# YooSungHyun/RNNTransducer

Measured on AMD Instinct MI355X. Metric: utterances/sec, higher is better.
Workload: dtype f32

## Files before the change

### include/rnnt_hip.h

```cpp
#ifndef RNNT_HIP_H_
#define RNNT_HIP_H_

#include <stddef.h>
#include <stdint.h>

#ifdef __cplusplus
extern "C" {
#endif

#define RNNT_HIP_ABI_VERSION 4

#define RNNT_OK 0
#define RNNT_ERR_INVALID (-1)
#define RNNT_ERR_LAUNCH (-2)
#define RNNT_ERR_UNSUPPORTED (-3)
#define RNNT_ERR_TIMEOUT (-4)

int rnnt_hip_version(void);
const char* rnnt_hip_last_error(void);
int rnnt_hip_device_cus(void);

enum {
  RNNT_K_GEMM = 0,
  RNNT_K_LSTM_FWD = 1,
  RNNT_K_LSTM_BWD = 2,
  RNNT_K_LSE = 3,
  RNNT_K_ALPHABETA = 4,
  RNNT_K_LATGRAD = 5,
  RNNT_K_MISC = 6,
  RNNT_K_GEMM_HP = 7,
  RNNT_K_HP_SPLIT = 8,
  RNNT_K_COUNT = 9
};
int rnnt_hip_prof_enable(int on);
int rnnt_hip_prof_collect(double* ms, double* work, int64_t* count, int nkinds);

int rnnt_hip_lstm_launch_log_enable(int on);
int64_t rnnt_hip_lstm_launch_log(char* buf, size_t n);

#define RNNT_GEMM_GELU_A 1u
#define RNNT_GEMM_GELU_B 2u
#define RNNT_GEMM_ACCUM 4u
#define RNNT_GEMM_MUL_DGELU 8u
#define RNNT_GEMM_EXACT_F32 16u
#define RNNT_GEMM_HP_F16 32u

typedef struct rnnt_gemm_desc {
  int64_t M, N, K;
  const float* A;
  int64_t a_div, a_so, a_si, a_sk;
  int32_t a_mc;
  const int64_t* a_rowidx;
  const float* B;
  int64_t b_sn, b_sk;
  float* C;
  int64_t c_div, c_so, c_si;
  const float* bias;
  const float* aux;
  uint32_t flags;
  void* workspace;
  size_t workspace_bytes;
} rnnt_gemm_desc;

size_t rnnt_hip_gemm_workspace_bytes(int64_t M, int64_t N, int64_t K);
int rnnt_hip_gemm_f32(const rnnt_gemm_desc* d, void* stream);

typedef struct rnnt_gemm_plan {
  int32_t mode;
  int32_t tile_m, tile_n;
  int32_t a_kc, b_kc;
  int32_t vec;
  int32_t tiles;
  int32_t splits, kchunk;
} rnnt_gemm_plan;
int rnnt_hip_gemm_plan(const rnnt_gemm_desc* d, rnnt_gemm_plan* out);

size_t rnnt_hip_hp_bytes(int64_t rows, int64_t K);
int rnnt_hip_hp_split(const float* x, int64_t rows, int64_t K, int64_t ld, int32_t transpose, int64_t src_rows, int64_t shift,
                      void* planes, uint32_t* amax, int32_t amax_given, void* stream);
int rnnt_hip_hp_split_both(const float* x, int64_t M, int64_t C, int64_t ld, const uint32_t* rowmax, const uint32_t* colmax,
                           void* planes_rm, void* planes_t, void* stream);
size_t rnnt_hip_gemm_hp_workspace_bytes(int64_t M, int64_t N, int64_t K);
int rnnt_hip_gemm_hp(const void* A, const uint32_t* a_amax, const void* B, const uint32_t* b_amax, int64_t M, int64_t N, int64_t K,
                     float* C, int64_t ldc, const float* bias, uint32_t flags, void* workspace, size_t workspace_bytes,
                     void* stream);

typedef struct rnnt_hp_problem {
  const void* A; const uint32_t* a_amax;
  const void* B; const uint32_t* b_amax;
  int64_t M, N, K;
  float* C; int64_t ldc;
  uint32_t flags;
} rnnt_hp_problem;
size_t rnnt_hip_gemm_hp_grouped_workspace_bytes(const rnnt_hp_problem* problems, int32_t n);
int rnnt_hip_gemm_hp_grouped(const rnnt_hp_problem* problems, int32_t n, uint32_t xcd_skip, void* workspace, size_t workspace_bytes,
                             void* stream);

#define RNNT_CELL_LSTM 0
#define RNNT_CELL_GRU 1
#define RNNT_CELL_RNN_TANH 2
#define RNNT_CELL_RNN_RELU 3

typedef struct rnnt_lstm_desc {
  int32_t T, B, I, H, D;
  int32_t cell;
  const int32_t* lens;
  const float* x;
  int64_t x_st, x_sb;
  const float* w_ih[2];
  const float* w_hh[2];
  const float* b_ih[2];
  const float* b_hh[2];
  float* y;
  float* y_drop;
  float dropout_p;
  uint64_t dropout_seed;
  float* gates;
  float* cst;
  float* aux;
  void* workspace;
  size_t workspace_bytes;
  uint32_t* status;
  float x_abs_bound;
  const int32_t* row_idx;
  int32_t n_rows;
} rnnt_lstm_desc;

size_t rnnt_hip_lstm_workspace_bytes(int32_t T, int32_t B, int32_t I, int32_t H, int32_t D);
int32_t rnnt_hip_lstm_max_batch(int32_t H, int32_t D, int32_t cell);
int32_t rnnt_hip_lstm_free_xcds(int32_t T, int32_t B, int32_t H, int32_t D, int32_t cell);
int32_t rnnt_hip_lstm_takes_row_idx(int32_t T, int32_t B, int32_t I, int32_t H, int32_t D, int32_t cell);
int rnnt_hip_lstm_fwd(const rnnt_lstm_desc* d, void* stream);

#define RNNT_PRECISION_FP32 0
#define RNNT_PRECISION_F16 1
int rnnt_hip_lstm_fwd_ex(const rnnt_lstm_desc* d, uint32_t precision, void* stream);
int32_t rnnt_hip_lstm_takes_f16(int32_t T, int32_t B, int32_t I, int32_t H, int32_t D, int32_t cell);

typedef struct rnnt_lstm_bwd_desc {
  rnnt_lstm_desc f;
  const float* dy;
  float* dx;
  float* dw_ih[2];
  float* dw_hh[2];
  float* db[2];
  float* db_hh[2];
  int32_t accumulate;
  int32_t phase;
  int32_t beside_recurrence;
} rnnt_lstm_bwd_desc;
#define RNNT_LSTM_BWD_ALL 0
#define RNNT_LSTM_BWD_RECUR 1
#define RNNT_LSTM_BWD_WEIGHTS 2

int rnnt_hip_lstm_bwd(const rnnt_lstm_bwd_desc* d, void* stream);
int rnnt_hip_lstm_bwd_ex(const rnnt_lstm_bwd_desc* d, uint32_t precision, void* stream);
int rnnt_hip_lstm_check(const void* workspace, void* stream);
int rnnt_hip_lstm_debug_read(const void* workspace, int32_t T, int32_t B, int32_t I, int32_t H, int32_t D,
                             uint64_t* out, int32_t nwg, void* stream);

size_t rnnt_hip_joint_loss_workspace_bytes(int32_t B, int32_t T, int32_t U1, int32_t V);
int rnnt_hip_joint_loss_fwd_bwd(const float* A, int64_t a_sb, int64_t a_st, const float* C, int64_t c_sb, int64_t c_su,
                                const float* bias, const int32_t* labels, const int32_t* t_lens,
                                const int32_t* u_lens, int32_t B, int32_t T, int32_t U1, int32_t V, int32_t blank,
                                float gscale, float* nll, float* dA, float* dC, void* workspace,
                                size_t workspace_bytes, void* stream);

int rnnt_hip_joint_loss_bwd(const float* A, int64_t a_sb, int64_t a_st, const float* C, int64_t c_sb, int64_t c_su,
                            const float* bias, const int32_t* labels, const int32_t* t_lens, const int32_t* u_lens,
                            int32_t B, int32_t T, int32_t U1, int32_t V, int32_t blank, float gscale, const float* gvec,
                            int32_t gvec_stride, float* dA, float* dC, void* workspace, size_t workspace_bytes, void* stream);
int rnnt_hip_scaled_sum_f32(const float* x, int32_t n, float scale, float* out, void* stream);

int rnnt_hip_joint_logits_fwd(const float* A, int64_t a_sb, int64_t a_st, const float* C, int64_t c_sb, int64_t c_su,
                              const float* bias, int32_t B, int32_t T, int32_t U1, int32_t V, float* logits,
                              void* stream);

int rnnt_hip_loss_from_logits_fwd_bwd(const float* logits, const int32_t* labels, const int32_t* t_lens,
                                      const int32_t* u_lens, int32_t B, int32_t T, int32_t U1, int32_t V,
                                      int32_t blank, float gscale, float* nll, float* grad, void* workspace,
                                      size_t workspace_bytes, void* stream);

int rnnt_hip_embedding_fwd(const float* W, const int64_t* idx, int64_t M, int32_t H, int32_t V, float* out, void* stream);

#define RNNT_DTYPE_F32 0
#define RNNT_DTYPE_F16 1
#define RNNT_DTYPE_BF16 2
int rnnt_hip_loss_from_logits_fwd_bwd_ex(const void* logits, int32_t dtype, const int32_t* labels, const int32_t* t_lens,
                                         const int32_t* u_lens, int32_t B, int32_t T, int32_t U1, int32_t V, int32_t blank,
                                         float gscale, float* nll, void* grad, void* workspace, size_t workspace_bytes,
                                         void* stream);

size_t rnnt_hip_joint_align_workspace_bytes(int32_t B, int32_t T, int32_t U1, int32_t V);
int rnnt_hip_joint_align(const float* A, int64_t a_sb, int64_t a_st, const float* C, int64_t c_sb, int64_t c_su,
                         const float* bias, const int32_t* labels, const int32_t* t_lens, const int32_t* u_lens,
                         int32_t B, int32_t T, int32_t U1, int32_t V, int32_t blank, int32_t* frames, double* score,
                         void* workspace, size_t workspace_bytes, void* stream);
int rnnt_hip_align_from_logits_ex(const void* logits, int32_t dtype, const int32_t* labels, const int32_t* t_lens,
                                  const int32_t* u_lens, int32_t B, int32_t T, int32_t U1, int32_t V, int32_t blank,
                                  int32_t* frames, double* score, void* workspace, size_t workspace_bytes, void* stream);

int rnnt_hip_adamw_step(float* p, const float* g, float* m, float* v, int64_t n, float lr, float beta1, float beta2, float eps,
                        float weight_decay, int64_t step, void* stream);
int rnnt_hip_adamw_step_ex(float* p, const float* g, float* m, float* v, int64_t n, float lr, float beta1, float beta2, float eps,
                           float weight_decay, int64_t step, float grad_scale, const uint32_t* guard, void* stream);

size_t rnnt_hip_colsum_workspace_bytes(int64_t M, int64_t N);
int rnnt_hip_colsum_f32(const float* X, int64_t M, int64_t N, int64_t ld, float* out, void* workspace,
                        size_t workspace_bytes, void* stream);
int rnnt_hip_colsum_f32_acc(const float* X, int64_t M, int64_t N, int64_t ld, float* out, void* workspace,
                            size_t workspace_bytes, void* stream);

int rnnt_hip_embedding_bwd(const float* dE, const int64_t* idx, int64_t M, int32_t H, int32_t V, int64_t padding_idx,
                           float* dW, void* stream);
int rnnt_hip_embedding_bwd_acc(const float* dE, const int64_t* idx, int64_t M, int32_t H, int32_t V, int64_t padding_idx,
                               float* dW, void* stream);

#define RNNT_DECODE_MAX_LAYERS 8
typedef struct rnnt_decode_desc {
  int32_t T, B, V;
  int32_t Hp, O, L;
  int32_t cell;
  int32_t blank, max_iters, max_out;
  const float* A;
  const int32_t* t_lens;
  const float* emb;
  const float* w_ih[RNNT_DECODE_MAX_LAYERS];
  const float* w_hh[RNNT_DECODE_MAX_LAYERS];
  const float* b_ih[RNNT_DECODE_MAX_LAYERS];
  const float* b_hh[RNNT_DECODE_MAX_LAYERS];
  const float* w_o;
  const float* b_o;
  const float* w_d;
  int64_t ld_d;
  int64_t* tokens;
  int32_t* ntok;
} rnnt_decode_desc;
int rnnt_hip_greedy_decode(const rnnt_decode_desc* d, void* stream);

typedef struct rnnt_prednet_step_desc {
  int32_t B, Hp, L, cell;
  const int64_t* tokens;
  const float* emb;
  const float* w_ih[RNNT_DECODE_MAX_LAYERS];
  const float* w_hh[RNNT_DECODE_MAX_LAYERS];
  const float* b_ih[RNNT_DECODE_MAX_LAYERS];
  const float* b_hh[RNNT_DECODE_MAX_LAYERS];
  const float* h_in;
  const float* c_in;
  float* h_out;
  float* c_out;
} rnnt_prednet_step_desc;
int rnnt_hip_prednet_step(const rnnt_prednet_step_desc* d, void* stream);

#define RNNT_BEAM_ST_OK 0
#define RNNT_BEAM_ST_CANDIDATES 1
#define RNNT_BEAM_ST_POPS 2
#define RNNT_BEAM_ST_STATES 3
#define RNNT_BEAM_ST_NODES 4
#define RNNT_BEAM_ST_LEN 5
#define RNNT_BEAM_NSTATS 6
typedef struct rnnt_beam_desc {
  int32_t T, B, V;
  int32_t Hp, O, L;
  int32_t cell, blank;
  int32_t beam, improved;
  double state_beam, expand_beam;
  int32_t max_candidates, max_pops, max_states, max_nodes, max_len;
  const float* A;
  const int32_t* t_lens;
  const float* emb;
  const float* w_ih[RNNT_DECODE_MAX_LAYERS];
  const float* w_hh[RNNT_DECODE_MAX_LAYERS];
  const float* b_ih[RNNT_DECODE_MAX_LAYERS];
  const float* b_hh[RNNT_DECODE_MAX_LAYERS];
  const float* w_o;
  const float* b_o;
  const float* w_d;
  int64_t ld_d;
  void* workspace;
  size_t workspace_bytes;
  int32_t* tokens;
  int32_t* lens;
  double* scores;
  int32_t* count;
  int32_t* status;
  int32_t* stats;
} rnnt_beam_desc;
size_t rnnt_hip_beam_workspace_bytes(const rnnt_beam_desc* d);
int rnnt_hip_beam_search(const rnnt_beam_desc* d, void* stream);

#define RNNT_STREAM_MAX_LAYERS 8
typedef struct rnnt_stream_rnn_desc {
  int32_t T, B, F, H, L, cell;
  int32_t O, V;
  const float* x;
  int64_t x_sb, x_st;
  const int32_t* lens;
  const float* w_ih[RNNT_STREAM_MAX_LAYERS];
  const float* w_hh[RNNT_STREAM_MAX_LAYERS];
  const float* b_ih[RNNT_STREAM_MAX_LAYERS];
  const float* b_hh[RNNT_STREAM_MAX_LAYERS];
  float* h;
  float* c;
  const float* w_o;
  const float* b_o;
  float* out;
  int64_t out_sb, out_st;
  const float* fc_w;
  int64_t ld_fc;
  const float* fc_b;
  float* A;
  void* workspace;
  size_t workspace_bytes;
} rnnt_stream_rnn_desc;
size_t rnnt_hip_stream_rnn_workspace_bytes(const rnnt_stream_rnn_desc* d);
int rnnt_hip_stream_rnn_chunk(const rnnt_stream_rnn_desc* d, void* stream);

typedef struct rnnt_stream_greedy_desc {
  int32_t T, B, V, Hp, O, L, cell;
  int32_t blank, max_iters, max_out;
  const float* A;
  const int32_t* lens;
  const float* emb;
  const float* w_ih[RNNT_DECODE_MAX_LAYERS];
  const float* w_hh[RNNT_DECODE_MAX_LAYERS];
  const float* b_ih[RNNT_DECODE_MAX_LAYERS];
  const float* b_hh[RNNT_DECODE_MAX_LAYERS];
  const float* w_o;
  const float* b_o;
  const float* w_d;
  int64_t ld_d;
  float* h;
  float* c;
  float* C;
  int64_t* last;
  int64_t* tokens;
  int32_t* ntok;
} rnnt_stream_greedy_desc;
int rnnt_hip_stream_greedy(const rnnt_stream_greedy_desc* d, void* stream);
int rnnt_hip_stream_greedy_reset(const rnnt_stream_greedy_desc* d, const int32_t* rows, int32_t n_rows, void* stream);

typedef struct rnnt_beam_stream_desc {
  int32_t T, B, V;
  int32_t Hp, O, L;
  int32_t cell, blank;
  int32_t beam, improved;
  double state_beam, expand_beam;
  int32_t max_candidates, max_pops, max_states, max_nodes, max_len;
  const float* A;
  const int32_t* lens;
  const float* emb;
  const float* w_ih[RNNT_DECODE_MAX_LAYERS];
  const float* w_hh[RNNT_DECODE_MAX_LAYERS];
  const float* b_ih[RNNT_DECODE_MAX_LAYERS];
  const float* b_hh[RNNT_DECODE_MAX_LAYERS];
  const float* w_o;
  const float* b_o;
  const float* w_d;
  int64_t ld_d;
  void* workspace;
  size_t workspace_bytes;
  int32_t* tokens;
  int32_t* out_lens;
  double* scores;
  int32_t* count;
  int32_t* status;
  int32_t* commit;
  int32_t* ncommit;
  int32_t* stats;
} rnnt_beam_stream_desc;
size_t rnnt_hip_beam_stream_workspace_bytes(const rnnt_beam_stream_desc* d);
int rnnt_hip_beam_stream_reset(const rnnt_beam_stream_desc* d, const int32_t* rows, int32_t n_rows, int32_t build_table,
                               void* stream);
int rnnt_hip_beam_stream_chunk(const rnnt_beam_stream_desc* d, void* stream);

typedef struct rnnt_greedy_timing {
  int32_t* frames;
  float* logp;
  const int64_t* frame_base;
} rnnt_greedy_timing;
int rnnt_hip_greedy_decode_timed(const rnnt_decode_desc* d, const rnnt_greedy_timing* timing, void* stream);
int rnnt_hip_stream_greedy_timed(const rnnt_stream_greedy_desc* d, const rnnt_greedy_timing* timing, void* stream);

typedef struct rnnt_beam_timing {
  int32_t* frames;
  int32_t* commit_frames;
} rnnt_beam_timing;
int rnnt_hip_beam_search_timed(const rnnt_beam_desc* d, const rnnt_beam_timing* timing, void* stream);
int rnnt_hip_beam_stream_chunk_timed(const rnnt_beam_stream_desc* d, const rnnt_beam_timing* timing, void* stream);

int rnnt_hip_frontend_norm_pad(const float* wav, int64_t ld, const int32_t* lens, int32_t B, int32_t pad, int64_t Lp,
                               int32_t normalize, float* out, void* stream);
int rnnt_hip_power_mel_log1p(const float* spec, int64_t M, int32_t n_bins, const float* fb, int32_t n_mels,
                             const int32_t* nframes, int32_t frames_per_utt, float* out, void* stream);

#ifdef __cplusplus
}
#endif
#endif
```

### rnntransducer_amd/_lib.py

```python
from __future__ import annotations

import ctypes as C
import os

_HERE = os.path.dirname(os.path.abspath(__file__))
LIB_PATH = os.environ.get("RNNT_HIP_LIB") or os.path.join(_HERE, "csrc", "librnnt_hip.so")
ABI_VERSION = 4

GEMM_GELU_A, GEMM_GELU_B, GEMM_ACCUM, GEMM_MUL_DGELU, GEMM_EXACT_F32 = 1, 2, 4, 8, 16
GEMM_HP_F16 = 32
PRECISION_FP32, PRECISION_F16 = 0, 1
CELL_LSTM, CELL_GRU, CELL_RNN_TANH, CELL_RNN_RELU = 0, 1, 2, 3

c_f32p = C.c_void_p
c_i64 = C.c_int64
c_i32 = C.c_int32


class GemmDesc(C.Structure):
    _fields_ = [("M", c_i64), ("N", c_i64), ("K", c_i64), ("A", C.c_void_p), ("a_div", c_i64), ("a_so", c_i64),
                ("a_si", c_i64), ("a_sk", c_i64), ("a_mc", c_i32), ("a_rowidx", C.c_void_p), ("B", C.c_void_p),
                ("b_sn", c_i64), ("b_sk", c_i64), ("C", C.c_void_p), ("c_div", c_i64), ("c_so", c_i64),
                ("c_si", c_i64), ("bias", C.c_void_p), ("aux", C.c_void_p), ("flags", C.c_uint32),
                ("workspace", C.c_void_p), ("workspace_bytes", C.c_size_t)]


class GemmPlan(C.Structure):
    _fields_ = [("mode", c_i32), ("tile_m", c_i32), ("tile_n", c_i32), ("a_kc", c_i32), ("b_kc", c_i32), ("vec", c_i32),
                ("tiles", c_i32), ("splits", c_i32), ("kchunk", c_i32)]


class LstmDesc(C.Structure):
    _fields_ = [("T", c_i32), ("B", c_i32), ("I", c_i32), ("H", c_i32), ("D", c_i32), ("cell", c_i32), ("lens", C.c_void_p),
                ("x", C.c_void_p), ("x_st", c_i64), ("x_sb", c_i64), ("w_ih", C.c_void_p * 2),
                ("w_hh", C.c_void_p * 2), ("b_ih", C.c_void_p * 2), ("b_hh", C.c_void_p * 2), ("y", C.c_void_p),
                ("y_drop", C.c_void_p), ("dropout_p", C.c_float), ("dropout_seed", C.c_uint64),
                ("gates", C.c_void_p), ("cst", C.c_void_p), ("aux", C.c_void_p), ("workspace", C.c_void_p),
                ("workspace_bytes", C.c_size_t), ("status", C.c_void_p), ("x_abs_bound", C.c_float), ("row_idx", C.c_void_p),
                ("n_rows", c_i32)]


class LstmBwdDesc(C.Structure):
    _fields_ = [("f", LstmDesc), ("dy", C.c_void_p), ("dx", C.c_void_p), ("dw_ih", C.c_void_p * 2),
                ("dw_hh", C.c_void_p * 2), ("db", C.c_void_p * 2), ("db_hh", C.c_void_p * 2), ("accumulate", c_i32), ("phase", c_i32),
                ("beside_recurrence", c_i32)]


class HpProblem(C.Structure):
    _fields_ = [("A", C.c_void_p), ("a_amax", C.c_void_p), ("B", C.c_void_p), ("b_amax", C.c_void_p), ("M", c_i64), ("N", c_i64),
                ("K", c_i64), ("C", C.c_void_p), ("ldc", c_i64), ("flags", C.c_uint32)]


DECODE_MAX_LAYERS = 8


class DecodeDesc(C.Structure):
    _fields_ = [("T", c_i32), ("B", c_i32), ("V", c_i32), ("Hp", c_i32), ("O", c_i32), ("L", c_i32), ("cell", c_i32),
                ("blank", c_i32), ("max_iters", c_i32), ("max_out", c_i32), ("A", C.c_void_p), ("t_lens", C.c_void_p), ("emb", C.c_void_p),
                ("w_ih", C.c_void_p * DECODE_MAX_LAYERS), ("w_hh", C.c_void_p * DECODE_MAX_LAYERS),
                ("b_ih", C.c_void_p * DECODE_MAX_LAYERS), ("b_hh", C.c_void_p * DECODE_MAX_LAYERS),
                ("w_o", C.c_void_p), ("b_o", C.c_void_p), ("w_d", C.c_void_p), ("ld_d", c_i64),
                ("tokens", C.c_void_p), ("ntok", C.c_void_p)]


class PrednetStepDesc(C.Structure):
    _fields_ = [("B", c_i32), ("Hp", c_i32), ("L", c_i32), ("cell", c_i32), ("tokens", C.c_void_p), ("emb", C.c_void_p),
                ("w_ih", C.c_void_p * DECODE_MAX_LAYERS), ("w_hh", C.c_void_p * DECODE_MAX_LAYERS),
                ("b_ih", C.c_void_p * DECODE_MAX_LAYERS), ("b_hh", C.c_void_p * DECODE_MAX_LAYERS),
                ("h_in", C.c_void_p), ("c_in", C.c_void_p), ("h_out", C.c_void_p), ("c_out", C.c_void_p)]


BEAM_STATUS = {1: ("A entries in one frame", "max_candidates"), 2: ("pops in one frame", "max_pops"),
               3: ("live prediction-net states", "max_states"), 4: ("prefix-tree nodes", "max_nodes"),
               5: ("tokens in a returned hypothesis", "max_len")}
BEAM_NSTATS = 6


class BeamDesc(C.Structure):
    _fields_ = [("T", c_i32), ("B", c_i32), ("V", c_i32), ("Hp", c_i32), ("O", c_i32), ("L", c_i32), ("cell", c_i32),
                ("blank", c_i32), ("beam", c_i32), ("improved", c_i32), ("state_beam", C.c_double), ("expand_beam", C.c_double),
                ("max_candidates", c_i32), ("max_pops", c_i32), ("max_states", c_i32), ("max_nodes", c_i32), ("max_len", c_i32),
                ("A", C.c_void_p), ("t_lens", C.c_void_p), ("emb", C.c_void_p),
                ("w_ih", C.c_void_p * DECODE_MAX_LAYERS), ("w_hh", C.c_void_p * DECODE_MAX_LAYERS),
                ("b_ih", C.c_void_p * DECODE_MAX_LAYERS), ("b_hh", C.c_void_p * DECODE_MAX_LAYERS),
                ("w_o", C.c_void_p), ("b_o", C.c_void_p), ("w_d", C.c_void_p), ("ld_d", c_i64),
                ("workspace", C.c_void_p), ("workspace_bytes", C.c_size_t), ("tokens", C.c_void_p), ("lens", C.c_void_p),
                ("scores", C.c_void_p), ("count", C.c_void_p), ("status", C.c_void_p), ("stats", C.c_void_p)]


STREAM_MAX_LAYERS = 8


class StreamRnnDesc(C.Structure):
    _fields_ = [("T", c_i32), ("B", c_i32), ("F", c_i32), ("H", c_i32), ("L", c_i32), ("cell", c_i32), ("O", c_i32), ("V", c_i32),
                ("x", C.c_void_p), ("x_sb", c_i64), ("x_st", c_i64), ("lens", C.c_void_p),
                ("w_ih", C.c_void_p * STREAM_MAX_LAYERS), ("w_hh", C.c_void_p * STREAM_MAX_LAYERS),
                ("b_ih", C.c_void_p * STREAM_MAX_LAYERS), ("b_hh", C.c_void_p * STREAM_MAX_LAYERS),
                ("h", C.c_void_p), ("c", C.c_void_p), ("w_o", C.c_void_p), ("b_o", C.c_void_p),
                ("out", C.c_void_p), ("out_sb", c_i64), ("out_st", c_i64), ("fc_w", C.c_void_p), ("ld_fc", c_i64),
                ("fc_b", C.c_void_p), ("A", C.c_void_p), ("workspace", C.c_void_p), ("workspace_bytes", C.c_size_t)]


class StreamGreedyDesc(C.Structure):
    _fields_ = [("T", c_i32), ("B", c_i32), ("V", c_i32), ("Hp", c_i32), ("O", c_i32), ("L", c_i32), ("cell", c_i32),
                ("blank", c_i32), ("max_iters", c_i32), ("max_out", c_i32), ("A", C.c_void_p), ("lens", C.c_void_p),
                ("emb", C.c_void_p), ("w_ih", C.c_void_p * DECODE_MAX_LAYERS), ("w_hh", C.c_void_p * DECODE_MAX_LAYERS),
                ("b_ih", C.c_void_p * DECODE_MAX_LAYERS), ("b_hh", C.c_void_p * DECODE_MAX_LAYERS),
                ("w_o", C.c_void_p), ("b_o", C.c_void_p), ("w_d", C.c_void_p), ("ld_d", c_i64),
                ("h", C.c_void_p), ("c", C.c_void_p), ("C", C.c_void_p), ("last", C.c_void_p),
                ("tokens", C.c_void_p), ("ntok", C.c_void_p)]


class BeamStreamDesc(C.Structure):
    _fields_ = [("T", c_i32), ("B", c_i32), ("V", c_i32), ("Hp", c_i32), ("O", c_i32), ("L", c_i32), ("cell", c_i32),
                ("blank", c_i32), ("beam", c_i32), ("improved", c_i32), ("state_beam", C.c_double), ("expand_beam", C.c_double),
                ("max_candidates", c_i32), ("max_pops", c_i32), ("max_states", c_i32), ("max_nodes", c_i32), ("max_len", c_i32),
                ("A", C.c_void_p), ("lens", C.c_void_p), ("emb", C.c_void_p),
                ("w_ih", C.c_void_p * DECODE_MAX_LAYERS), ("w_hh", C.c_void_p * DECODE_MAX_LAYERS),
                ("b_ih", C.c_void_p * DECODE_MAX_LAYERS), ("b_hh", C.c_void_p * DECODE_MAX_LAYERS),
                ("w_o", C.c_void_p), ("b_o", C.c_void_p), ("w_d", C.c_void_p), ("ld_d", c_i64),
                ("workspace", C.c_void_p), ("workspace_bytes", C.c_size_t), ("tokens", C.c_void_p), ("out_lens", C.c_void_p),
                ("scores", C.c_void_p), ("count", C.c_void_p), ("status", C.c_void_p), ("commit", C.c_void_p),
                ("ncommit", C.c_void_p), ("stats", C.c_void_p)]


class GreedyTiming(C.Structure):
    _fields_ = [("frames", C.c_void_p), ("logp", C.c_void_p), ("frame_base", C.c_void_p)]


class BeamTiming(C.Structure):
    _fields_ = [("frames", C.c_void_p), ("commit_frames", C.c_void_p)]


SYMBOLS = {
    "rnnt_hip_version": (C.c_int, []),
    "rnnt_hip_last_error": (C.c_char_p, []),
    "rnnt_hip_device_cus": (C.c_int, []),
    "rnnt_hip_prof_enable": (C.c_int, [C.c_int]),
    "rnnt_hip_prof_collect": (C.c_int, [C.c_void_p, C.c_void_p, C.c_void_p, C.c_int]),
    "rnnt_hip_lstm_launch_log_enable": (C.c_int, [C.c_int]),
    "rnnt_hip_lstm_launch_log": (c_i64, [C.c_char_p, C.c_size_t]),
    "rnnt_hip_gemm_workspace_bytes": (C.c_size_t, [c_i64, c_i64, c_i64]),
    "rnnt_hip_gemm_f32": (C.c_int, [C.POINTER(GemmDesc), C.c_void_p]),
    "rnnt_hip_gemm_plan": (C.c_int, [C.POINTER(GemmDesc), C.POINTER(GemmPlan)]),
    "rnnt_hip_hp_bytes": (C.c_size_t, [c_i64, c_i64]),
    "rnnt_hip_hp_split": (C.c_int, [C.c_void_p, c_i64, c_i64, c_i64, c_i32, c_i64, c_i64, C.c_void_p, C.c_void_p, c_i32, C.c_void_p]),
    "rnnt_hip_gemm_hp_workspace_bytes": (C.c_size_t, [c_i64, c_i64, c_i64]),
    "rnnt_hip_gemm_hp": (C.c_int, [C.c_void_p, C.c_void_p, C.c_void_p, C.c_void_p, c_i64, c_i64, c_i64, C.c_void_p, c_i64, C.c_void_p,
                                  C.c_uint32, C.c_void_p, C.c_size_t, C.c_void_p]),
    "rnnt_hip_hp_split_both": (C.c_int, [C.c_void_p, c_i64, c_i64, c_i64, C.c_void_p, C.c_void_p, C.c_void_p, C.c_void_p, C.c_void_p]),
    "rnnt_hip_gemm_hp_grouped_workspace_bytes": (C.c_size_t, [C.POINTER(HpProblem), c_i32]),
    "rnnt_hip_gemm_hp_grouped": (C.c_int, [C.POINTER(HpProblem), c_i32, C.c_uint32, C.c_void_p, C.c_size_t, C.c_void_p]),
    "rnnt_hip_lstm_workspace_bytes": (C.c_size_t, [c_i32] * 5),
    "rnnt_hip_lstm_max_batch": (c_i32, [c_i32, c_i32, c_i32]),
    "rnnt_hip_lstm_free_xcds": (c_i32, [c_i32] * 5),
    "rnnt_hip_lstm_takes_row_idx": (c_i32, [c_i32] * 6),
    "rnnt_hip_lstm_fwd": (C.c_int, [C.POINTER(LstmDesc), C.c_void_p]),
    "rnnt_hip_lstm_fwd_ex": (C.c_int, [C.POINTER(LstmDesc), C.c_uint32, C.c_void_p]),
    "rnnt_hip_lstm_takes_f16": (c_i32, [c_i32] * 6),
    "rnnt_hip_lstm_bwd": (C.c_int, [C.POINTER(LstmBwdDesc), C.c_void_p]),
    "rnnt_hip_lstm_bwd_ex": (C.c_int, [C.POINTER(LstmBwdDesc), C.c_uint32, C.c_void_p]),
    "rnnt_hip_lstm_check": (C.c_int, [C.c_void_p, C.c_void_p]),
    "rnnt_hip_lstm_debug_read": (C.c_int, [C.c_void_p, c_i32, c_i32, c_i32, c_i32, c_i32, C.c_void_p, c_i32, C.c_void_p]),
    "rnnt_hip_joint_loss_workspace_bytes": (C.c_size_t, [c_i32] * 4),
    "rnnt_hip_joint_loss_fwd_bwd": (C.c_int, [C.c_void_p, c_i64, c_i64, C.c_void_p, c_i64, c_i64, C.c_void_p, C.c_void_p,
                                               C.c_void_p, C.c_void_p, c_i32, c_i32, c_i32, c_i32, c_i32, C.c_float,
                                               C.c_void_p, C.c_void_p, C.c_void_p, C.c_void_p, C.c_size_t, C.c_void_p]),
    "rnnt_hip_joint_loss_bwd": (C.c_int, [C.c_void_p, c_i64, c_i64, C.c_void_p, c_i64, c_i64, C.c_void_p, C.c_void_p,
                                           C.c_void_p, C.c_void_p, c_i32, c_i32, c_i32, c_i32, c_i32, C.c_float, C.c_void_p, c_i32,
                                           C.c_void_p, C.c_void_p, C.c_void_p, C.c_size_t, C.c_void_p]),
    "rnnt_hip_scaled_sum_f32": (C.c_int, [C.c_void_p, c_i32, C.c_float, C.c_void_p, C.c_void_p]),
    "rnnt_hip_joint_logits_fwd": (C.c_int, [C.c_void_p, c_i64, c_i64, C.c_void_p, c_i64, c_i64, C.c_void_p, c_i32, c_i32,
                                             c_i32, c_i32, C.c_void_p, C.c_void_p]),
    "rnnt_hip_loss_from_logits_fwd_bwd": (C.c_int, [C.c_void_p, C.c_void_p, C.c_void_p, C.c_void_p, c_i32, c_i32, c_i32,
                                                     c_i32, c_i32, C.c_float, C.c_void_p, C.c_void_p, C.c_void_p,
                                                     C.c_size_t, C.c_void_p]),
    "rnnt_hip_loss_from_logits_fwd_bwd_ex": (C.c_int, [C.c_void_p, c_i32, C.c_void_p, C.c_void_p, C.c_void_p, c_i32, c_i32,
                                                        c_i32, c_i32, c_i32, C.c_float, C.c_void_p, C.c_void_p,
                                                        C.c_void_p, C.c_size_t, C.c_void_p]),
    "rnnt_hip_joint_align_workspace_bytes": (C.c_size_t, [c_i32] * 4),
    "rnnt_hip_joint_align": (C.c_int, [C.c_void_p, c_i64, c_i64, C.c_void_p, c_i64, c_i64, C.c_void_p, C.c_void_p, C.c_void_p,
                                       C.c_void_p, c_i32, c_i32, c_i32, c_i32, c_i32, C.c_void_p, C.c_void_p, C.c_void_p,
                                       C.c_size_t, C.c_void_p]),
    "rnnt_hip_align_from_logits_ex": (C.c_int, [C.c_void_p, c_i32, C.c_void_p, C.c_void_p, C.c_void_p, c_i32, c_i32, c_i32, c_i32,
                                                c_i32, C.c_void_p, C.c_void_p, C.c_void_p, C.c_size_t, C.c_void_p]),
    "rnnt_hip_adamw_step": (C.c_int, [C.c_void_p, C.c_void_p, C.c_void_p, C.c_void_p, c_i64, C.c_float, C.c_float, C.c_float,
                                     C.c_float, C.c_float, c_i64, C.c_void_p]),
    "rnnt_hip_adamw_step_ex": (C.c_int, [C.c_void_p, C.c_void_p, C.c_void_p, C.c_void_p, c_i64, C.c_float, C.c_float, C.c_float,
                                        C.c_float, C.c_float, c_i64, C.c_float, C.c_void_p, C.c_void_p]),
    "rnnt_hip_embedding_fwd": (C.c_int, [C.c_void_p, C.c_void_p, c_i64, c_i32, c_i32, C.c_void_p, C.c_void_p]),
    "rnnt_hip_colsum_workspace_bytes": (C.c_size_t, [c_i64, c_i64]),
    "rnnt_hip_colsum_f32": (C.c_int, [C.c_void_p, c_i64, c_i64, c_i64, C.c_void_p, C.c_void_p, C.c_size_t, C.c_void_p]),
    "rnnt_hip_colsum_f32_acc": (C.c_int, [C.c_void_p, c_i64, c_i64, c_i64, C.c_void_p, C.c_void_p, C.c_size_t, C.c_void_p]),
    "rnnt_hip_embedding_bwd": (C.c_int, [C.c_void_p, C.c_void_p, c_i64, c_i32, c_i32, c_i64, C.c_void_p, C.c_void_p]),
    "rnnt_hip_embedding_bwd_acc": (C.c_int, [C.c_void_p, C.c_void_p, c_i64, c_i32, c_i32, c_i64, C.c_void_p, C.c_void_p]),
    "rnnt_hip_greedy_decode": (C.c_int, [C.POINTER(DecodeDesc), C.c_void_p]),
    "rnnt_hip_prednet_step": (C.c_int, [C.POINTER(PrednetStepDesc), C.c_void_p]),
    "rnnt_hip_beam_workspace_bytes": (C.c_size_t, [C.POINTER(BeamDesc)]),
    "rnnt_hip_beam_search": (C.c_int, [C.POINTER(BeamDesc), C.c_void_p]),
    "rnnt_hip_stream_rnn_workspace_bytes": (C.c_size_t, [C.POINTER(StreamRnnDesc)]),
    "rnnt_hip_stream_rnn_chunk": (C.c_int, [C.POINTER(StreamRnnDesc), C.c_void_p]),
    "rnnt_hip_stream_greedy": (C.c_int, [C.POINTER(StreamGreedyDesc), C.c_void_p]),
    "rnnt_hip_stream_greedy_reset": (C.c_int, [C.POINTER(StreamGreedyDesc), C.c_void_p, c_i32, C.c_void_p]),
    "rnnt_hip_beam_stream_workspace_bytes": (C.c_size_t, [C.POINTER(BeamStreamDesc)]),
    "rnnt_hip_beam_stream_reset": (C.c_int, [C.POINTER(BeamStreamDesc), C.c_void_p, c_i32, c_i32, C.c_void_p]),
    "rnnt_hip_beam_stream_chunk": (C.c_int, [C.POINTER(BeamStreamDesc), C.c_void_p]),
    "rnnt_hip_greedy_decode_timed": (C.c_int, [C.POINTER(DecodeDesc), C.POINTER(GreedyTiming), C.c_void_p]),
    "rnnt_hip_stream_greedy_timed": (C.c_int, [C.POINTER(StreamGreedyDesc), C.POINTER(GreedyTiming), C.c_void_p]),
    "rnnt_hip_beam_search_timed": (C.c_int, [C.POINTER(BeamDesc), C.POINTER(BeamTiming), C.c_void_p]),
    "rnnt_hip_beam_stream_chunk_timed": (C.c_int, [C.POINTER(BeamStreamDesc), C.POINTER(BeamTiming), C.c_void_p]),
    "rnnt_hip_frontend_norm_pad": (C.c_int, [C.c_void_p, c_i64, C.c_void_p, c_i32, c_i32, c_i64, c_i32, C.c_void_p, C.c_void_p]),
    "rnnt_hip_power_mel_log1p": (C.c_int, [C.c_void_p, c_i64, c_i32, C.c_void_p, c_i32, C.c_void_p, c_i32, C.c_void_p, C.c_void_p]),
}

KERNEL_KINDS = ["gemm_f32_kernel", "lstm_fwd_kernel", "lstm_bwd_kernel", "lse_kernel", "alphabeta_kernel",
                "lattice_grad_kernel", "misc", "gemm_hp_kernel", "hp_split_kernels"]

_lib = None


class RnntHipError(RuntimeError):
    pass


def lib():
    global _lib
    if _lib is None:
        if not os.path.exists(LIB_PATH):
            raise RnntHipError(
                f"{LIB_PATH} not found: build it with `python -m rnntransducer_amd.csrc.build` "
                "(or __graft_entry__.build()).  rnntransducer_amd has no non-HIP execution path.")
        handle = C.CDLL(LIB_PATH)
        for name, (res, args) in SYMBOLS.items():
            fn = getattr(handle, name)
            fn.restype = res
            fn.argtypes = args
        if handle.rnnt_hip_version() != ABI_VERSION:
            raise RnntHipError(f"{LIB_PATH} reports ABI version {handle.rnnt_hip_version()}, this package binds version {ABI_VERSION}: "
                               "rebuild it with `python -m rnntransducer_amd.csrc.build`")
        _lib = handle
    return _lib


def check(rc: int, what: str = "") -> None:
    if rc != 0:
        msg = lib().rnnt_hip_last_error().decode("utf-8", "replace")
        if rc == -1:
            raise ValueError(f"{what}: {msg}")
        raise RnntHipError(f"{what}: rc={rc}: {msg}")
```

### rnntransducer_amd/csrc/common.hpp

```cpp
#pragma once
#include <hip/hip_runtime.h>
#include <stdarg.h>
#include <stdint.h>
#include <stdio.h>

#include <atomic>

#include "rnnt_hip.h"

namespace rnnt {

void set_error(const char* fmt, ...);

#define RNNT_CHECK_ARG(cond, ...)      \
  do {                                 \
    if (!(cond)) {                     \
      ::rnnt::set_error(__VA_ARGS__);  \
      return RNNT_ERR_INVALID;         \
    }                                  \
  } while (0)

#define RNNT_CHECK_HIP(expr)                                                          \
  do {                                                                                \
    hipError_t e_ = (expr);                                                           \
    if (e_ != hipSuccess) {                                                           \
      ::rnnt::set_error("%s failed: %s (%s:%d)", #expr, hipGetErrorString(e_), __FILE__, __LINE__); \
      return RNNT_ERR_LAUNCH;                                                         \
    }                                                                                 \
  } while (0)

#define RNNT_CHECK_LAUNCH() RNNT_CHECK_HIP(hipGetLastError())

struct ProfScope {
  ProfScope(int kind, double work, hipStream_t s);
  ~ProfScope();
  int kind_;
  double work_;
  hipStream_t stream_;
  void* start_;
};

extern std::atomic<bool> g_launch_log_on;
void launch_log_note(const void* kernel, hipStream_t s);

static inline int64_t ceil_div(int64_t a, int64_t b) { return (a + b - 1) / b; }

int launch_colsum(const float* X, long M, long N, long ld, float* out, void* ws, size_t ws_bytes, hipStream_t s, int accumulate = 0);

size_t hp_plane_bytes(int64_t rows, int64_t K);
int hp_colmax(const float* x, int64_t rows, int64_t C, int64_t ld, uint32_t* amax, hipStream_t s);
int hp_split(const float* x, int64_t rows, int64_t K, int64_t ld, uint32_t* amax, void* planes, hipStream_t s, const int* rowidx = nullptr);
int hp_split_t(const float* x, int64_t R, int64_t K, int64_t ld, int64_t Ksrc, int64_t shift, const uint32_t* amax, void* planes,
               hipStream_t s, const int* kidx = nullptr);
int hp_split_both(const float* x, int64_t M, int64_t C, int64_t ld, const uint32_t* rowmax, const uint32_t* colmax, void* planes_rm,
                  void* planes_t, hipStream_t s, const int* rowidx = nullptr);
size_t hp_gemm_workspace_bytes(int64_t M, int64_t N, int64_t K);
int hp_gemm(const void* A, const uint32_t* a_amax, const void* B, const uint32_t* b_amax, int64_t M, int64_t N, int64_t K, float* C,
            int64_t c_div, int64_t c_so, int64_t c_si, const float* bias, unsigned flags, void* workspace, size_t workspace_bytes,
            hipStream_t s, const int* a_rowidx = nullptr, int64_t a_plane_rows = 0, const int* c_rowidx = nullptr);
struct HpProblem {
  const void* A; const uint32_t* a_amax; const void* B; const uint32_t* b_amax;
  int64_t M, N, K;
  float* C; int64_t ldc;
  unsigned flags;
};
constexpr int HP_GROUP_MAX = 4;
size_t hp_gemm_grouped_workspace_bytes(const int64_t* MN, int n);
int hp_gemm_grouped(const HpProblem* pr, int n, unsigned xcd_skip, unsigned* counter, void* workspace, size_t workspace_bytes,
                    hipStream_t s, unsigned* status = nullptr);
constexpr size_t HPQ_HEADER_BYTES = 256;
static inline size_t align_up(size_t a, size_t b) { return (a + b - 1) / b * b; }

__device__ __forceinline__ float gelu_tanh(float x) {
  const float k0 = 0.7978845608028654f, k1 = 0.044715f;
  float u = k0 * (x + k1 * x * x * x);
  return 0.5f * x * (1.0f + tanhf(u));
}
__device__ __forceinline__ float dgelu_tanh(float x) {
  const float k0 = 0.7978845608028654f, k1 = 0.044715f;
  float x2 = x * x;
  float u = k0 * (x + k1 * x * x2);
  float th = tanhf(u);
  float du = k0 * (1.0f + 3.0f * k1 * x2);
  return 0.5f * (1.0f + th) + 0.5f * x * (1.0f - th * th) * du;
}

__device__ __forceinline__ float sigmoidf_(float x) { return 1.0f / (1.0f + expf(-x)); }
__device__ __forceinline__ float tanh_e(float x) { return 1.0f - 2.0f / (expf(2.0f * x) + 1.0f); }
__device__ __forceinline__ float sigmoid_hw(float x) { return __builtin_amdgcn_rcpf(1.0f + __expf(-x)); }
__device__ __forceinline__ float tanh_hw(float x) { return 1.0f - 2.0f * __builtin_amdgcn_rcpf(__expf(2.0f * x) + 1.0f); }

typedef float f32x4 __attribute__((ext_vector_type(4)));
typedef float f32x16 __attribute__((ext_vector_type(16)));
typedef __bf16 bf16x8 __attribute__((ext_vector_type(8)));
typedef unsigned u32x4 __attribute__((ext_vector_type(4)));
typedef unsigned u32x2 __attribute__((ext_vector_type(2)));

template <int NPL>
__device__ __forceinline__ void split_pair(float xe, float xo, unsigned (&pk)[NPL]) {
  constexpr unsigned SEL = 0x07060302u;
  const unsigned ue = __float_as_uint(xe), uo = __float_as_uint(xo);
  pk[0] = __builtin_amdgcn_perm(uo, ue, SEL);
  const float re = xe - __uint_as_float(ue & 0xffff0000u), ro = xo - __uint_as_float(uo & 0xffff0000u);
  unsigned ure = __float_as_uint(re), uro = __float_as_uint(ro);
  if constexpr (NPL == 2) {
    ure += 0x8000u;
    uro += 0x8000u;
  }
  pk[1] = __builtin_amdgcn_perm(uro, ure, SEL);
  if constexpr (NPL == 3) {
    const float le = re - __uint_as_float(ure & 0xffff0000u), lo = ro - __uint_as_float(uro & 0xffff0000u);
    pk[2] = __builtin_amdgcn_perm(__float_as_uint(lo), __float_as_uint(le), SEL);
  }
}

__device__ __forceinline__ void split8(const f32x4& lo4, const f32x4& hi4, bf16x8 (&piece)[3]) {
  unsigned q0[3], q1[3], q2[3], q3[3];
  split_pair<3>(lo4[0], lo4[1], q0);
  split_pair<3>(lo4[2], lo4[3], q1);
  split_pair<3>(hi4[0], hi4[1], q2);
  split_pair<3>(hi4[2], hi4[3], q3);
#pragma unroll
  for (int pl = 0; pl < 3; ++pl) piece[pl] = __builtin_bit_cast(bf16x8, (u32x4){q0[pl], q1[pl], q2[pl], q3[pl]});
}

}
```

### rnntransducer_amd/csrc/gemm_hp.hip

```cpp
#include "common.hpp"

#include <stdlib.h>

namespace rnnt {
namespace {

typedef _Float16 f16x8 __attribute__((ext_vector_type(8)));
typedef __attribute__((address_space(3))) void lds_void;

constexpr int HP_BM = 256, HP_BN = 256, HP_BK = 32;
constexpr int HP_STAGE = (HP_BM + HP_BN) * 128;
constexpr int HP_RSRC = 0x00027000;

__device__ __forceinline__ float hp_scale_from_amax(unsigned amax_bits) {
  int eb = (int)((amax_bits >> 23) & 255u);
  if (eb == 0) return 1.0f;
  eb = eb < 15 ? 15 : eb;
  return __uint_as_float((unsigned)(268 - eb) << 23);
}
__device__ __forceinline__ float hp_inv_scale_from_amax(unsigned amax_bits) {
  int eb = (int)((amax_bits >> 23) & 255u);
  if (eb == 0) return 1.0f;
  eb = eb < 15 ? 15 : eb;
  return __uint_as_float((unsigned)(eb - 14) << 23);
}

__global__ void __launch_bounds__(256) hp_colmax_kernel(const float* __restrict__ x, long rows, int C, long ld, long rows_per_chunk,
                                                        unsigned* __restrict__ out) {
  const int c = blockIdx.x * 256 + threadIdx.x;
  if (c >= C) return;
  const long r0 = (long)blockIdx.y * rows_per_chunk, r1 = min(rows, r0 + rows_per_chunk);
  unsigned m = 0;
  for (long r = r0; r < r1; ++r) m = max(m, __float_as_uint(x[r * ld + c]) & 0x7fffffffu);
  if (m != 0) atomicMax(out + c, m);
}

__device__ __forceinline__ void hp_split8(const float (&x)[8], float scale, u32x4& hi, u32x4& lo) {
  f16x8 h, l;
#pragma unroll
  for (int e = 0; e < 8; ++e) {
    const float v = x[e] * scale;
    const _Float16 a = (_Float16)v;
    h[e] = a;
    l[e] = (_Float16)(v - (float)a);
  }
  hi = __builtin_bit_cast(u32x4, h);
  lo = __builtin_bit_cast(u32x4, l);
}

__global__ void __launch_bounds__(256) hp_split_kernel(const float* __restrict__ x, long rows, int K, long ld, unsigned* __restrict__ amax,
                                                       char* __restrict__ out, const int* __restrict__ rowidx) {
  const int Kp = (K + 31) & ~31, cpr = Kp >> 3;
  const int lane = threadIdx.x & 63;
  const bool vec = (ld & 3) == 0 && (reinterpret_cast<uintptr_t>(x) & 15) == 0;
  for (long ri = (long)blockIdx.x * 4 + (threadIdx.x >> 6); ri < rows; ri += (long)gridDim.x * 4) {
    const long r = rowidx ? (long)rowidx[ri] : ri;
    const float* row = x + r * ld;
    unsigned m = 0;
    for (int c = lane; c < cpr; c += 64) {
      const int k = 8 * c;
      if (vec && k + 7 < K) {
        const u32x4 a = *reinterpret_cast<const u32x4*>(row + k), b = *reinterpret_cast<const u32x4*>(row + k + 4);
#pragma unroll
        for (int e = 0; e < 4; ++e) m = max(m, max(a[e] & 0x7fffffffu, b[e] & 0x7fffffffu));
      } else {
#pragma unroll
        for (int e = 0; e < 8; ++e)
          if (k + e < K) m = max(m, __float_as_uint(row[k + e]) & 0x7fffffffu);
      }
    }
#pragma unroll
    for (int o = 32; o > 0; o >>= 1) m = max(m, (unsigned)__shfl_xor((int)m, o));
    if (lane == 0) amax[r] = m;
    const float scale = hp_scale_from_amax(m);
    for (int c = lane; c < cpr; c += 64) {
      const int k = 8 * c;
      float v[8];
      if (vec && k + 7 < K) {
        const f32x4 a = *reinterpret_cast<const f32x4*>(row + k), b = *reinterpret_cast<const f32x4*>(row + k + 4);
        v[0] = a[0]; v[1] = a[1]; v[2] = a[2]; v[3] = a[3]; v[4] = b[0]; v[5] = b[1]; v[6] = b[2]; v[7] = b[3];
      } else {
#pragma unroll
        for (int e = 0; e < 8; ++e) v[e] = (k + e < K) ? row[k + e] : 0.f;
      }
      u32x4 hi, lo;
      hp_split8(v, scale, hi, lo);
      char* dst = out + (r * (Kp >> 5) + (c >> 2)) * 128 + 16 * (c & 3);
      *reinterpret_cast<u32x4*>(dst) = hi;
      *reinterpret_cast<u32x4*>(dst + 64) = lo;
    }
  }
}

__global__ void __launch_bounds__(256) hp_split_t_kernel(const float* __restrict__ x, int R, int K, long ld, int Ksrc, int shift,
                                                         const unsigned* __restrict__ amax, char* __restrict__ out,
                                                         const int* __restrict__ kidx) {
  __shared__ float tile[32][257];
  const int kb = blockIdx.x, r0 = blockIdx.y * 256;
  const int tid = threadIdx.x;
  const bool vec = (ld & 3) == 0 && (reinterpret_cast<uintptr_t>(x) & 15) == 0;
#pragma unroll
  for (int q = 0; q < 8; ++q) {
    const int kk = 4 * q + (tid >> 6);
    const int kdst = kb * 32 + kk;
    const int ksrc = (kidx ? (kdst < K ? kidx[kdst] : 0) : kdst) + shift;
    const int c = 4 * (tid & 63);
    f32x4 v = {0.f, 0.f, 0.f, 0.f};
    if (kdst < K && ksrc >= 0 && ksrc < Ksrc) {
      const float* src = x + (long)ksrc * ld + r0 + c;
      if (vec && r0 + c + 3 < R) {
        v = *reinterpret_cast<const f32x4*>(src);
      } else {
#pragma unroll
        for (int e = 0; e < 4; ++e)
          if (r0 + c + e < R) v[e] = src[e];
      }
    }
#pragma unroll
    for (int e = 0; e < 4; ++e) tile[kk][c + e] = v[e];
  }
  __syncthreads();
  const int Kp32 = (K + 31) >> 5;
#pragma unroll
  for (int ps = 0; ps < 4; ++ps) {
    const int rl = (tid >> 2) + 64 * ps, ch = tid & 3;
    if (r0 + rl < R) {
      float v[8];
#pragma unroll
      for (int e = 0; e < 8; ++e) v[e] = tile[8 * ch + e][rl];
      u32x4 hi, lo;
      hp_split8(v, hp_scale_from_amax(amax[r0 + rl]), hi, lo);
      char* dst = out + ((long)(r0 + rl) * Kp32 + kb) * 128 + 16 * ch;
      *reinterpret_cast<u32x4*>(dst) = hi;
      *reinterpret_cast<u32x4*>(dst + 64) = lo;
    }
  }
}

__global__ void __launch_bounds__(256) hp_split_both_kernel(const float* __restrict__ x, int M, int C, long ld, const unsigned* __restrict__ rowmax,
                                                            const unsigned* __restrict__ colmax, char* __restrict__ out_rm, char* __restrict__ out_t,
                                                            const int* __restrict__ rowidx) {
  __shared__ float tile[32][257];
  const int kb = blockIdx.x, c0 = blockIdx.y * 256;
  const int tid = threadIdx.x;
  const int Cp = (C + 31) & ~31;
  const bool vec = (ld & 3) == 0 && (reinterpret_cast<uintptr_t>(x) & 15) == 0;
#pragma unroll
  for (int q = 0; q < 4; ++q) {
    const int row = 8 * q + (tid >> 5), col = 8 * (tid & 31);
    const int ri = kb * 32 + row, c = c0 + col;
    const int r = (rowidx && ri < M) ? rowidx[ri] : ri;
    float v[8] = {0.f, 0.f, 0.f, 0.f, 0.f, 0.f, 0.f, 0.f};
    if (ri < M && c < C) {
      const float* src = x + (long)r * ld + c;
      if (vec && c + 7 < C) {
        const f32x4 a = *reinterpret_cast<const f32x4*>(src), b = *reinterpret_cast<const f32x4*>(src + 4);
        v[0] = a[0]; v[1] = a[1]; v[2] = a[2]; v[3] = a[3]; v[4] = b[0]; v[5] = b[1]; v[6] = b[2]; v[7] = b[3];
      } else {
#pragma unroll
        for (int e = 0; e < 8; ++e)
          if (c + e < C) v[e] = src[e];
      }
    }
    if (ri < M && c < Cp) {
      u32x4 hi, lo;
      hp_split8(v, hp_scale_from_amax(rowmax[r]), hi, lo);
      char* dst = out_rm + ((long)r * (Cp >> 5) + (c >> 5)) * 128 + 16 * ((c >> 3) & 3);
      *reinterpret_cast<u32x4*>(dst) = hi;
      *reinterpret_cast<u32x4*>(dst + 64) = lo;
    }
#pragma unroll
    for (int e = 0; e < 8; ++e) tile[row][col + e] = v[e];
  }
  __syncthreads();
  const int Mp32 = (M + 31) >> 5;
#pragma unroll
  for (int ps = 0; ps < 4; ++ps) {
    const int rl = (tid >> 2) + 64 * ps, ch = tid & 3;
    if (c0 + rl < C) {
      float v[8];
#pragma unroll
      for (int e = 0; e < 8; ++e) v[e] = tile[8 * ch + e][rl];
      u32x4 hi, lo;
      hp_split8(v, hp_scale_from_amax(colmax[c0 + rl]), hi, lo);
      char* dst = out_t + ((long)(c0 + rl) * Mp32 + kb) * 128 + 16 * ch;
      *reinterpret_cast<u32x4*>(dst) = hi;
      *reinterpret_cast<u32x4*>(dst + 64) = lo;
    }
  }
}

struct HpGemmK {
  int M, N, nkt;
  const char* A; unsigned a_pitch, a_bytes;
  const char* B; unsigned b_pitch, b_bytes;
  const unsigned* a_amax; const unsigned* b_amax;
  float* C; int c_div; long c_so, c_si;
  const float* bias;
  unsigned flags;
  int splits, kt_per_split;
  float* slab;
  int tiles_m, tiles_n;
  int group_m;
  const int* a_rowidx;
  const int* c_rowidx;
};

__device__ __forceinline__ int hp_xcd_remap(int bid, int n) {
  const int q = n / 8, r = n % 8, xcd = bid % 8;
  return (xcd < r ? xcd * (q + 1) : r * (q + 1) + (xcd - r) * q) + bid / 8;
}

template <bool F16>
__device__ __forceinline__ void hp_tile256(const HpGemmK& p, const int bid, const int z, char* lds) {
  const int tid = threadIdx.x, lane = tid & 63;
  const int wave = __builtin_amdgcn_readfirstlane(tid >> 6);
  const int wr = wave >> 2, wc = wave & 3;
  const int m0 = (bid % p.tiles_m) * HP_BM, n0 = (bid / p.tiles_m) * HP_BN;

  const __amdgpu_buffer_rsrc_t ra = __builtin_amdgcn_make_buffer_rsrc(const_cast<char*>(p.A), 0, (int)p.a_bytes, HP_RSRC);
  const __amdgpu_buffer_rsrc_t rb = __builtin_amdgcn_make_buffer_rsrc(const_cast<char*>(p.B), 0, (int)p.b_bytes, HP_RSRC);

  unsigned va[4], vb[4];
  {
    const int src_slot = (lane & 7) ^ (((lane >> 4) & 3) | ((wave & 1) << 2));
#pragma unroll
    for (int j = 0; j < 4; ++j) {
      const int row = (8 * j + wave) * 8 + (lane >> 3);
      int ma = min(m0 + row, p.M - 1);
      const int nb = min(n0 + row, p.N - 1);
      if (p.a_rowidx) ma = p.a_rowidx[ma];
      va[j] = (unsigned)ma * p.a_pitch + 16u * src_slot;
      vb[j] = (unsigned)nb * p.b_pitch + 16u * src_slot;
    }
  }
  auto stage = [&](int buf, int kt) {
    char* base = lds + buf * HP_STAGE;
    const int koff = kt * 128;
#pragma unroll
    for (int j = 0; j < 4; ++j) {
      __builtin_amdgcn_raw_ptr_buffer_load_lds(ra, (lds_void*)(base + (8 * j + wave) * 1024), 16, va[j], koff, 0, 0);
      __builtin_amdgcn_raw_ptr_buffer_load_lds(rb, (lds_void*)(base + HP_BM * 128 + (8 * j + wave) * 1024), 16, vb[j], koff, 0, 0);
    }
  };

  const int frag0 = (lane & 15) * 128 + 16 * ((lane >> 4) ^ ((lane & 15) >> 1));
  const int a_base = wr * (128 * 128) + frag0;
  const int b_base = HP_BM * 128 + wc * (64 * 128) + frag0;

  f32x4 acc[8][4];
#pragma unroll
  for (int i = 0; i < 8; ++i)
#pragma unroll
    for (int j = 0; j < 4; ++j) acc[i][j] = (f32x4){0.f, 0.f, 0.f, 0.f};

  const int kt0 = z * p.kt_per_split;
  const int nk = min(p.nkt - kt0, p.kt_per_split);

  stage(0, kt0);
  asm volatile("s_waitcnt vmcnt(0)" ::: "memory");
  __syncthreads();
  for (int kt = 0; kt < nk; ++kt) {
    const int cur = kt & 1;
#ifndef HP_DBG_NO_DMA
    if (kt + 1 < nk) stage(cur ^ 1, kt0 + kt + 1);
#endif
    const char* sb = lds + cur * HP_STAGE;
    f16x8 a[4][2], b[2][2];
#ifdef HP_DBG_NO_LDSREAD
    auto load_a = [&](int mq) {
#pragma unroll
      for (int i = 0; i < 4; ++i) { asm volatile("" : "+v"(a[i][0]), "+v"(a[i][1])); }
    };
    auto load_b = [&](int nq) {
#pragma unroll
      for (int j = 0; j < 2; ++j) { asm volatile("" : "+v"(b[j][0]), "+v"(b[j][1])); }
    };
#else
    auto load_a = [&](int mq) {
#pragma unroll
      for (int i = 0; i < 4; ++i) {
        a[i][0] = *reinterpret_cast<const f16x8*>(sb + (a_base + (4 * mq + i) * 2048));
        if constexpr (!F16) a[i][1] = *reinterpret_cast<const f16x8*>(sb + ((a_base ^ 64) + (4 * mq + i) * 2048));
      }
    };
    auto load_b = [&](int nq) {
#pragma unroll
      for (int j = 0; j < 2; ++j) {
        b[j][0] = *reinterpret_cast<const f16x8*>(sb + (b_base + (2 * nq + j) * 2048));
        if constexpr (!F16) b[j][1] = *reinterpret_cast<const f16x8*>(sb + ((b_base ^ 64) + (2 * nq + j) * 2048));
      }
    };
#endif
    auto mma = [&](int mq, int nq) {
#pragma unroll
      for (int i = 0; i < 4; ++i)
#pragma unroll
        for (int j = 0; j < 2; ++j) {
          f32x4 c = acc[4 * mq + i][2 * nq + j];
          if constexpr (!F16) {
            c = __builtin_amdgcn_mfma_f32_16x16x32_f16(a[i][1], b[j][0], c, 0, 0, 0);
            c = __builtin_amdgcn_mfma_f32_16x16x32_f16(a[i][0], b[j][1], c, 0, 0, 0);
          }
          c = __builtin_amdgcn_mfma_f32_16x16x32_f16(a[i][0], b[j][0], c, 0, 0, 0);
          acc[4 * mq + i][2 * nq + j] = c;
        }
    };
#ifndef HP_DBG_NO_MFMA
    load_a(0); load_b(0); mma(0, 0);
    load_b(1); mma(0, 1);
    load_a(1); mma(1, 1);
    load_b(0); mma(1, 0);
#endif
    __builtin_amdgcn_sched_barrier(0);
#ifndef HP_DBG_NO_BARRIER
    __syncthreads();
#endif
  }
  const int mode = p.splits > 1 ? 0 : ((p.flags & RNNT_GEMM_ACCUM) ? 2 : 1);
  float* slab = p.splits > 1 ? p.slab + (long)z * p.M * p.N : nullptr;
  float bias_v[4], sb[4];
#pragma unroll
  for (int j = 0; j < 4; ++j) {
    const int n = n0 + wc * 64 + j * 16 + (lane & 15);
    bias_v[j] = (mode != 0 && p.bias && n < p.N) ? p.bias[n] : 0.f;
    sb[j] = hp_inv_scale_from_amax(p.b_amax[min(n, p.N - 1)]);
  }
#pragma unroll
  for (int i = 0; i < 8; ++i) {
#pragma unroll
    for (int reg = 0; reg < 4; ++reg) {
      const int m = m0 + wr * 128 + i * 16 + 4 * (lane >> 4) + reg;
      const bool mok = m < p.M;
      const int mc = mok ? m : 0;
      const float sa = hp_inv_scale_from_amax(p.a_amax[p.a_rowidx ? p.a_rowidx[mc] : mc]);
      const int mo = p.c_rowidx ? p.c_rowidx[mc] : mc;
      float* crow = mode == 0 ? slab + (long)mc * p.N : p.C + (long)(mo / p.c_div) * p.c_so + (long)(mo % p.c_div) * p.c_si;
      float old[4] = {0.f, 0.f, 0.f, 0.f};
      if (mode == 2) {
#pragma unroll
        for (int j = 0; j < 4; ++j) {
          const int n = n0 + wc * 64 + j * 16 + (lane & 15);
          if (mok && n < p.N) old[j] = crow[n];
        }
      }
#pragma unroll
      for (int j = 0; j < 4; ++j) {
        const int n = n0 + wc * 64 + j * 16 + (lane & 15);
        if (mok && n < p.N) crow[n] = acc[i][j][reg] * sa * sb[j] + bias_v[j] + old[j];
      }
    }
  }
}

__device__ __forceinline__ int hp_grouped_tile(int idx, int tiles_m, int tiles_n, int group_m) {
  const int band = group_m * tiles_n;
  const int g = idx / band, r = idx - g * band;
  const int m_first = g * group_m;
  const int gm = min(tiles_m - m_first, group_m);
  const int n = r / gm, m = m_first + (r - n * gm);
  return n * tiles_m + m;
}

template <bool F16>
__global__ void __launch_bounds__(512, 1) gemm_hp_kernel(const HpGemmK p) {
  extern __shared__ __attribute__((aligned(16))) char lds[];
  int bid = hp_xcd_remap(blockIdx.x, p.tiles_m * p.tiles_n);
  if (p.group_m > 0) bid = hp_grouped_tile(bid, p.tiles_m, p.tiles_n, p.group_m);
  hp_tile256<F16>(p, bid, blockIdx.y, lds);
}

constexpr int HPQ_MAX = 4;
struct HpGemmQ {
  HpGemmK prob[HPQ_MAX];
  int unit_end[HPQ_MAX];
  int nprob;
  unsigned xcd_skip;
  unsigned* counter;
};

template <bool F16>
__global__ void __launch_bounds__(512, 1) gemm_hpq_kernel(const HpGemmQ q) {
  extern __shared__ __attribute__((aligned(16))) char lds[];
  unsigned xcc;
  asm volatile("s_getreg_b32 %0, hwreg(HW_REG_XCC_ID)" : "=s"(xcc));
  xcc &= 7u;
  if ((q.xcd_skip >> xcc) & 1u) return;
  const unsigned allow = ~q.xcd_skip & 0xffu;
  const int nq = __builtin_popcount(allow);
  const int mine = __builtin_popcount(allow & ((1u << xcc) - 1u));
  int* next = reinterpret_cast<int*>(lds + 2 * HP_STAGE);
  const int total = q.unit_end[q.nprob - 1];
  for (int hop = 0; hop < nq; ++hop) {
    const int qi = (mine + hop) % nq;
    const int lo = (int)((long)total * qi / nq), hi = (int)((long)total * (qi + 1) / nq);
    while (true) {
      if (threadIdx.x == 0) {
        const int got = lo + (int)atomicAdd(q.counter + qi, 1u);
        *next = got;
        if (got < hi) atomicAdd(q.counter + 8, 1u);
      }
      __syncthreads();
      const int u = __builtin_amdgcn_readfirstlane(*next);
      __syncthreads();
      if (u >= hi) break;
      int pi = 0;
      while (u >= q.unit_end[pi]) ++pi;
      const HpGemmK& p = q.prob[pi];
      const int local = u - (pi ? q.unit_end[pi - 1] : 0);
      const int tn = local % p.tiles_n, z = (local / p.tiles_n) % p.splits, tm = local / (p.tiles_n * p.splits);
      hp_tile256<F16>(p, tn * p.tiles_m + tm, z, lds);
    }
  }
}

__global__ void hpq_check_kernel(unsigned* counter, unsigned total, unsigned* status) {
  if (counter[8] != total) {
    counter[9] = 1u;
    if (status) __hip_atomic_store(status, 2u, __ATOMIC_RELAXED, __HIP_MEMORY_SCOPE_AGENT);
  }
}

__global__ void __launch_bounds__(256) hp_splitk_reduce_kernel(const HpGemmK p) {
  const long total = (long)p.M * p.N;
  for (long i = (long)blockIdx.x * 256 + threadIdx.x; i < total; i += (long)gridDim.x * 256) {
    const int m = (int)(i / p.N), n = (int)(i % p.N);
    float s = 0.f;
    for (int z = 0; z < p.splits; ++z) s += p.slab[(long)z * total + i];
    if (p.bias) s += p.bias[n];
    const int mo = p.c_rowidx ? p.c_rowidx[m] : m;
    const long off = (long)(mo / p.c_div) * p.c_so + (long)(mo % p.c_div) * p.c_si + n;
    if (p.flags & RNNT_GEMM_ACCUM) s += p.C[off];
    p.C[off] = s;
  }
}

}

size_t hp_plane_bytes(int64_t rows, int64_t K) { return (size_t)rows * (size_t)ceil_div(K, 32) * 128; }

int hp_colmax(const float* x, int64_t rows, int64_t C, int64_t ld, uint32_t* amax, hipStream_t s) {
  RNNT_CHECK_HIP(hipMemsetAsync(amax, 0, (size_t)C * 4, s));
  if (rows == 0 || C == 0) return RNNT_OK;
  long chunks = ceil_div(2048, ceil_div(C, 256));
  if (chunks > ceil_div(rows, 64)) chunks = ceil_div(rows, 64);
  if (chunks < 1) chunks = 1;
  const long rpc = ceil_div(rows, chunks);
  ProfScope prof(RNNT_K_HP_SPLIT, 4.0 * (double)rows * (double)C, s);
  hipLaunchKernelGGL(hp_colmax_kernel, dim3((unsigned)ceil_div(C, 256), (unsigned)ceil_div(rows, rpc)), dim3(256), 0, s, x, (long)rows, (int)C,
                     (long)ld, rpc, amax);
  RNNT_CHECK_LAUNCH();
  return RNNT_OK;
}

int hp_split(const float* x, int64_t rows, int64_t K, int64_t ld, uint32_t* amax, void* planes, hipStream_t s, const int* rowidx) {
  if (rows == 0) return RNNT_OK;
  const long blocks = ceil_div(rows, 4);
  ProfScope prof(RNNT_K_HP_SPLIT, 8.0 * (double)rows * (double)K, s);
  hipLaunchKernelGGL(hp_split_kernel, dim3((unsigned)(blocks < 8192 ? blocks : 8192)), dim3(256), 0, s, x, (long)rows, (int)K, (long)ld, amax,
                     (char*)planes, rowidx);
  RNNT_CHECK_LAUNCH();
  return RNNT_OK;
}

int hp_split_t(const float* x, int64_t R, int64_t K, int64_t ld, int64_t Ksrc, int64_t shift, const uint32_t* amax, void* planes,
               hipStream_t s, const int* kidx) {
  if (R == 0 || K == 0) return RNNT_OK;
  ProfScope prof(RNNT_K_HP_SPLIT, 8.0 * (double)R * (double)K, s);
  hipLaunchKernelGGL(hp_split_t_kernel, dim3((unsigned)ceil_div(K, 32), (unsigned)ceil_div(R, 256)), dim3(256), 0, s, x, (int)R, (int)K, (long)ld,
                     (int)Ksrc, (int)shift, amax, (char*)planes, kidx);
  RNNT_CHECK_LAUNCH();
  return RNNT_OK;
}

int hp_split_both(const float* x, int64_t M, int64_t C, int64_t ld, const uint32_t* rowmax, const uint32_t* colmax, void* planes_rm,
                  void* planes_t, hipStream_t s, const int* rowidx) {
  if (M == 0 || C == 0) return RNNT_OK;
  ProfScope prof(RNNT_K_HP_SPLIT, 12.0 * (double)M * (double)C, s);
  hipLaunchKernelGGL(hp_split_both_kernel, dim3((unsigned)ceil_div(M, 32), (unsigned)ceil_div(C, 256)), dim3(256), 0, s, x, (int)M, (int)C, (long)ld,
                     rowmax, colmax, (char*)planes_rm, (char*)planes_t, rowidx);
  RNNT_CHECK_LAUNCH();
  return RNNT_OK;
}

size_t hp_gemm_workspace_bytes(int64_t M, int64_t N, int64_t K) {
  const long tiles = ceil_div(M, HP_BM) * ceil_div(N, HP_BN);
  const long nkt = ceil_div(K, HP_BK);
  if (tiles >= 192 || nkt < 64) return 0;
  long want = ceil_div(256, tiles);
  if (want > nkt / 32) want = nkt / 32;
  if (want > 32) want = 32;
  return want >= 2 ? (size_t)want * M * N * 4 : 0;
}

int hp_gemm(const void* A, const uint32_t* a_amax, const void* B, const uint32_t* b_amax, int64_t M, int64_t N, int64_t K, float* C,
            int64_t c_div, int64_t c_so, int64_t c_si, const float* bias, unsigned flags, void* workspace, size_t workspace_bytes,
            hipStream_t s, const int* a_rowidx, int64_t a_plane_rows, const int* c_rowidx) {
  RNNT_CHECK_ARG(A && B && C && a_amax && b_amax, "gemm_hp: null operand");
  RNNT_CHECK_ARG(!a_rowidx || a_plane_rows >= M, "gemm_hp: a gathered A operand needs the row count of its planes");
  RNNT_CHECK_ARG(M >= 1 && N >= 1 && K >= 1 && M < (1ll << 31) && N < (1ll << 31) && K < (1ll << 31), "gemm_hp: bad dims");
  RNNT_CHECK_ARG(c_div >= 1, "gemm_hp: c_div must be >= 1");
  RNNT_CHECK_ARG(((reinterpret_cast<uintptr_t>(A) | reinterpret_cast<uintptr_t>(B)) & 127) == 0, "gemm_hp: planes must be 128-byte aligned");
  HpGemmK k;
  k.M = (int)M; k.N = (int)N; k.nkt = (int)ceil_div(K, HP_BK);
  const size_t ab = hp_plane_bytes(a_rowidx ? a_plane_rows : M, K), bb = hp_plane_bytes(N, K);
  RNNT_CHECK_ARG(ab < (1ull << 32) && bb < (1ull << 32), "gemm_hp: an operand exceeds the 4 GB a buffer resource addresses");
  k.A = (const char*)A; k.a_pitch = (unsigned)k.nkt * 128u; k.a_bytes = (unsigned)ab;
  k.B = (const char*)B; k.b_pitch = (unsigned)k.nkt * 128u; k.b_bytes = (unsigned)bb;
  k.a_amax = a_amax; k.b_amax = b_amax;
  k.C = C; k.c_div = (int)(c_div > 0x7fffffff ? 0x7fffffff : c_div); k.c_so = c_so; k.c_si = c_si;
  k.bias = bias; k.flags = flags;
  k.a_rowidx = a_rowidx; k.c_rowidx = c_rowidx;
  const bool f16 = (flags & RNNT_GEMM_HP_F16) != 0u;
  k.tiles_m = (int)ceil_div(M, HP_BM); k.tiles_n = (int)ceil_div(N, HP_BN);
  const int tiles = k.tiles_m * k.tiles_n;
  {
    static const int env_gm = getenv("RNNT_GEMM_HP_GROUP_M") ? atoi(getenv("RNNT_GEMM_HP_GROUP_M")) : -1;
    k.group_m = env_gm >= 0 ? env_gm : (tiles >= 256 ? 8 : 4);
  }
  int splits = 1;
  if (workspace && tiles < 192 && k.nkt >= 64) {
    long want = ceil_div(256, tiles);
    const long by_ws = (long)(workspace_bytes / ((size_t)M * N * 4));
    if (want > k.nkt / 32) want = k.nkt / 32;
    if (want > by_ws) want = by_ws;
    if (want > 32) want = 32;
    if (want >= 2) splits = (int)want;
  }
  k.kt_per_split = (int)ceil_div(k.nkt, splits);
  splits = (int)ceil_div(k.nkt, k.kt_per_split);
  k.splits = splits;
  k.slab = (float*)workspace;
  if (f16) RNNT_CHECK_HIP(hipFuncSetAttribute((const void*)gemm_hp_kernel<true>, hipFuncAttributeMaxDynamicSharedMemorySize, 2 * HP_STAGE));
  else RNNT_CHECK_HIP(hipFuncSetAttribute((const void*)gemm_hp_kernel<false>, hipFuncAttributeMaxDynamicSharedMemorySize, 2 * HP_STAGE));
  {
    ProfScope prof(RNNT_K_GEMM_HP, 2.0 * (double)M * (double)N * (double)K, s);
    if (f16) hipLaunchKernelGGL(gemm_hp_kernel<true>, dim3(tiles, splits), dim3(512), 2 * HP_STAGE, s, k);
    else hipLaunchKernelGGL(gemm_hp_kernel<false>, dim3(tiles, splits), dim3(512), 2 * HP_STAGE, s, k);
    RNNT_CHECK_LAUNCH();
    if (splits > 1) {
      const long blocks = ceil_div((long)M * N, 256);
      hipLaunchKernelGGL(hp_splitk_reduce_kernel, dim3((unsigned)(blocks < 2048 ? blocks : 2048)), dim3(256), 0, s, k);
      RNNT_CHECK_LAUNCH();
    }
  }
  return RNNT_OK;
}

constexpr int HPQ_SPLIT_CAP = 8;
size_t hp_gemm_grouped_workspace_bytes(const int64_t* MN, int n) {
  size_t total = 0;
  for (int i = 0; i < n; ++i) total += align_up((size_t)HPQ_SPLIT_CAP * (size_t)MN[i] * 4, 256);
  return total;
}

int hp_gemm_grouped(const HpProblem* pr, int n, unsigned xcd_skip, unsigned* counter, void* workspace, size_t workspace_bytes,
                    hipStream_t s, unsigned* status) {
  RNNT_CHECK_ARG(pr && n >= 1 && n <= HPQ_MAX && counter, "gemm_hp grouped: 1..%d problems and a counter word", HPQ_MAX);
  RNNT_CHECK_ARG((xcd_skip & 0xffu) != 0xffu, "gemm_hp grouped: xcd_skip leaves no XCD");
  const bool f16 = (pr[0].flags & RNNT_GEMM_HP_F16) != 0u;
  for (int i = 1; i < n; ++i)
    RNNT_CHECK_ARG(((pr[i].flags & RNNT_GEMM_HP_F16) != 0u) == f16, "gemm_hp grouped: the problems of one launch share RNNT_GEMM_HP_F16");
  HpGemmQ q = {};
  q.nprob = n; q.xcd_skip = xcd_skip; q.counter = counter;
  int xcds = 0;
  for (int x = 0; x < 8; ++x) xcds += !((xcd_skip >> x) & 1u);
  const long workers = 32l * xcds;
  long total_kt = 0;
  double flops = 0.0;
  for (int i = 0; i < n; ++i) {
    const HpProblem& a = pr[i];
    RNNT_CHECK_ARG(a.A && a.B && a.C && a.a_amax && a.b_amax, "gemm_hp grouped: null operand (problem %d)", i);
    RNNT_CHECK_ARG(a.M >= 1 && a.N >= 1 && a.K >= 1 && a.M < (1ll << 31) && a.N < (1ll << 31) && a.K < (1ll << 31) && a.ldc >= a.N,
                   "gemm_hp grouped: bad dims (problem %d)", i);
    RNNT_CHECK_ARG(((reinterpret_cast<uintptr_t>(a.A) | reinterpret_cast<uintptr_t>(a.B)) & 127) == 0, "gemm_hp grouped: planes must be 128-byte aligned");
    HpGemmK& k = q.prob[i];
    k.M = (int)a.M; k.N = (int)a.N; k.nkt = (int)ceil_div(a.K, HP_BK);
    const size_t ab = hp_plane_bytes(a.M, a.K), bb = hp_plane_bytes(a.N, a.K);
    RNNT_CHECK_ARG(ab < (1ull << 32) && bb < (1ull << 32), "gemm_hp grouped: an operand exceeds the 4 GB a buffer resource addresses");
    k.A = (const char*)a.A; k.a_pitch = (unsigned)k.nkt * 128u; k.a_bytes = (unsigned)ab;
    k.B = (const char*)a.B; k.b_pitch = (unsigned)k.nkt * 128u; k.b_bytes = (unsigned)bb;
    k.a_amax = a.a_amax; k.b_amax = a.b_amax;
    k.C = a.C; k.c_div = 1; k.c_so = a.ldc; k.c_si = 0;
    k.bias = nullptr; k.flags = a.flags;
    k.a_rowidx = k.c_rowidx = nullptr;
    k.tiles_m = (int)ceil_div(a.M, HP_BM); k.tiles_n = (int)ceil_div(a.N, HP_BN);
    total_kt += (long)k.tiles_m * k.tiles_n * k.nkt;
    flops += 2.0 * (double)a.M * (double)a.N * (double)a.K;
  }
  long chunk = ceil_div(total_kt, 4 * workers);
  if (chunk < 32) chunk = 32;
  size_t off = 0;
  int units = 0;
  for (int i = 0; i < n; ++i) {
    HpGemmK& k = q.prob[i];
    long splits = ceil_div(k.nkt, chunk);
    if (splits > HPQ_SPLIT_CAP) splits = HPQ_SPLIT_CAP;
    const size_t per = (size_t)k.M * k.N * 4;
    while (splits > 1 && (!workspace || off + align_up((size_t)splits * per, 256) > workspace_bytes)) --splits;
    k.kt_per_split = (int)ceil_div(k.nkt, splits);
    k.splits = (int)ceil_div(k.nkt, k.kt_per_split);
    k.slab = k.splits > 1 ? reinterpret_cast<float*>((char*)workspace + off) : nullptr;
    if (k.splits > 1) off += align_up((size_t)k.splits * per, 256);
    units += k.tiles_m * k.tiles_n * k.splits;
    q.unit_end[i] = units;
  }
  RNNT_CHECK_HIP(hipMemsetAsync(counter, 0, 64, s));
  const int lds = 2 * HP_STAGE + 16;
  const void* qk = f16 ? (const void*)gemm_hpq_kernel<true> : (const void*)gemm_hpq_kernel<false>;
  RNNT_CHECK_HIP(hipFuncSetAttribute(qk, hipFuncAttributeMaxDynamicSharedMemorySize, lds));
  {
    ProfScope prof(RNNT_K_GEMM_HP, flops, s);
    int cus = 0, dev = 0;
    if (hipGetDevice(&dev) != hipSuccess || hipDeviceGetAttribute(&cus, hipDeviceAttributeMultiprocessorCount, dev) != hipSuccess || cus < 8) cus = 256;
    const dim3 grid(!xcd_skip && units < cus ? units : cus);
    if (f16) hipLaunchKernelGGL(gemm_hpq_kernel<true>, grid, dim3(512), lds, s, q);
    else hipLaunchKernelGGL(gemm_hpq_kernel<false>, grid, dim3(512), lds, s, q);
    RNNT_CHECK_LAUNCH();
    hipLaunchKernelGGL(hpq_check_kernel, dim3(1), dim3(1), 0, s, counter, (unsigned)units, status);
    RNNT_CHECK_LAUNCH();
    for (int i = 0; i < n; ++i)
      if (q.prob[i].splits > 1) {
        const long blocks = ceil_div((long)q.prob[i].M * q.prob[i].N, 256);
        hipLaunchKernelGGL(hp_splitk_reduce_kernel, dim3((unsigned)(blocks < 2048 ? blocks : 2048)), dim3(256), 0, s, q.prob[i]);
        RNNT_CHECK_LAUNCH();
      }
  }
  return RNNT_OK;
}

}

using namespace rnnt;

extern "C" size_t rnnt_hip_hp_bytes(int64_t rows, int64_t K) {
  if (rows < 0 || K < 0) return 0;
  return hp_plane_bytes(rows, K);
}

extern "C" int rnnt_hip_hp_split(const float* x, int64_t rows, int64_t K, int64_t ld, int32_t transpose, int64_t src_rows, int64_t shift,
                                 void* planes, uint32_t* amax, int32_t amax_given, void* stream) {
  RNNT_CHECK_ARG(x && planes && amax && rows >= 0 && K >= 0, "hp_split: bad arguments");
  RNNT_CHECK_ARG((reinterpret_cast<uintptr_t>(planes) & 127) == 0, "hp_split: planes must be 128-byte aligned");
  hipStream_t s = (hipStream_t)stream;
  if (!transpose) {
    RNNT_CHECK_ARG(ld >= K, "hp_split: ld < K");
    RNNT_CHECK_ARG(!amax_given, "hp_split: the row-major split computes its row maxima itself");
    return hp_split(x, rows, K, ld, amax, planes, s);
  }
  RNNT_CHECK_ARG(ld >= rows && src_rows >= 1, "hp_split: transposed source is (src_rows x >= rows), ld >= rows");
  if (!amax_given)
    if (int rc = hp_colmax(x, src_rows, rows, ld, amax, s)) return rc;
  return hp_split_t(x, rows, K, ld, src_rows, shift, amax, planes, s);
}

extern "C" size_t rnnt_hip_gemm_hp_workspace_bytes(int64_t M, int64_t N, int64_t K) {
  if (M < 1 || N < 1 || K < 1) return 0;
  return hp_gemm_workspace_bytes(M, N, K);
}

extern "C" int rnnt_hip_gemm_hp(const void* A, const uint32_t* a_amax, const void* B, const uint32_t* b_amax, int64_t M, int64_t N,
                                int64_t K, float* C, int64_t ldc, const float* bias, uint32_t flags, void* workspace,
                                size_t workspace_bytes, void* stream) {
  RNNT_CHECK_ARG(ldc >= N, "gemm_hp: ldc < N");
  return hp_gemm(A, a_amax, B, b_amax, M, N, K, C, 1, ldc, 0, bias, flags, workspace, workspace_bytes, (hipStream_t)stream);
}

static_assert(sizeof(rnnt_hp_problem) == sizeof(HpProblem), "rnnt_hp_problem mirrors HpProblem");

extern "C" size_t rnnt_hip_gemm_hp_grouped_workspace_bytes(const rnnt_hp_problem* problems, int32_t n) {
  if (!problems || n < 1 || n > HP_GROUP_MAX) return 0;
  int64_t mn[HP_GROUP_MAX];
  for (int i = 0; i < n; ++i) mn[i] = problems[i].M * problems[i].N;
  return 256 + hp_gemm_grouped_workspace_bytes(mn, n);
}

extern "C" int rnnt_hip_gemm_hp_grouped(const rnnt_hp_problem* problems, int32_t n, uint32_t xcd_skip, void* workspace,
                                        size_t workspace_bytes, void* stream) {
  RNNT_CHECK_ARG(problems && n >= 1 && n <= HP_GROUP_MAX, "gemm_hp grouped: 1..%d problems", HP_GROUP_MAX);
  RNNT_CHECK_ARG(workspace && workspace_bytes >= 256 && (reinterpret_cast<uintptr_t>(workspace) & 255) == 0,
                 "gemm_hp grouped: workspace of >= 256 bytes, 256-byte aligned");
  HpProblem pr[HP_GROUP_MAX];
  for (int i = 0; i < n; ++i) {
    const rnnt_hp_problem& a = problems[i];
    pr[i] = HpProblem{a.A, a.a_amax, a.B, a.b_amax, a.M, a.N, a.K, a.C, a.ldc, a.flags};
  }
  return hp_gemm_grouped(pr, n, xcd_skip, reinterpret_cast<unsigned*>(workspace), (char*)workspace + 256, workspace_bytes - 256,
                         (hipStream_t)stream);
}

extern "C" int rnnt_hip_hp_split_both(const float* x, int64_t M, int64_t C, int64_t ld, const uint32_t* rowmax, const uint32_t* colmax,
                                      void* planes_rm, void* planes_t, void* stream) {
  RNNT_CHECK_ARG(x && rowmax && colmax && planes_rm && planes_t && M >= 0 && C >= 0 && ld >= C, "hp_split_both: bad arguments");
  RNNT_CHECK_ARG(M < (1ll << 31) && C < (1ll << 31), "hp_split_both: dims must fit 31 bits");
  RNNT_CHECK_ARG(((reinterpret_cast<uintptr_t>(planes_rm) | reinterpret_cast<uintptr_t>(planes_t)) & 127) == 0, "hp_split_both: planes must be 128-byte aligned");
  return hp_split_both(x, M, C, ld, rowmax, colmax, planes_rm, planes_t, (hipStream_t)stream);
}
```

### rnntransducer_amd/csrc/lstm_layer.hip

```cpp
#include "lstm_shared.hpp"

#include <string.h>

namespace rnnt {
namespace {

__global__ void db_reduce_kernel(const float* __restrict__ part, int rows_per_dir, int H, int ngate, float* __restrict__ o0,
                                 float* __restrict__ o1, int accumulate, float* __restrict__ p0 = nullptr,
                                 float* __restrict__ p1 = nullptr) {
  const int c = blockIdx.x * 256 + threadIdx.x, d = blockIdx.y;
  if (c >= 4 * H || (c & 3) >= ngate) return;
  const float* src = part + (long)d * rows_per_dir * 4 * H + c;
  float s = 0.f;
  for (int r = 0; r < rows_per_dir; ++r) s += src[(long)r * 4 * H];
  float* o = (d ? o1 : o0) + (c & 3) * H + (c >> 2);
  *o = accumulate ? *o + s : s;
  float* q = d ? p1 : p0;
  if (q) {
    q += (c & 3) * H + (c >> 2);
    *q = accumulate ? *q + s : s;
  }
}
__global__ void permute_w_kernel(const float* __restrict__ w0, const float* __restrict__ w1, int H, int I, int ngate,
                                 float* __restrict__ out) {
  const long per = (long)4 * H * I;
  const long idx = (long)blockIdx.x * 256 + threadIdx.x;
  const int d = blockIdx.y;
  if (idx >= per) return;
  const int k = (int)(idx % I), r = (int)(idx / I);
  const float* w = d ? w1 : w0;
  out[d * per + idx] = (r & 3) < ngate ? w[(long)((r & 3) * H + (r >> 2)) * I + k] : 0.f;
}
__global__ void __launch_bounds__(256) zero_padded_rows_kernel(float* __restrict__ x, const int* __restrict__ lens, int T, int B, int I) {
  const int lane = threadIdx.x & 63;
  const long nrow = (long)T * B;
  const long nw = ((long)gridDim.x * blockDim.x) >> 6;
  for (long r = ((long)blockIdx.x * blockDim.x + threadIdx.x) >> 6; r < nrow; r += nw) {
    if ((int)(r / B) < lens[r % B]) continue;
    float* row = x + r * I;
    for (int i = lane; i < I; i += 64) row[i] = 0.f;
  }
}
__global__ void unpermute_w_kernel(const float* __restrict__ in, int H, int I, long in_dir_stride, int ngate,
                                   float* __restrict__ o0, float* __restrict__ o1, int accumulate, float* __restrict__ p0 = nullptr,
                                   float* __restrict__ p1 = nullptr) {
  const long per = (long)4 * H * I;
  const long idx = (long)blockIdx.x * 256 + threadIdx.x;
  const int d = blockIdx.y;
  if (idx >= per) return;
  const int k = (int)(idx % I), r = (int)(idx / I);
  float* o = d ? o1 : o0;
  if ((r & 3) < ngate) {
    const long off = (long)((r & 3) * H + (r >> 2)) * I + k;
    const float v = in[d * in_dir_stride + idx];
    o[off] = accumulate ? o[off] + v : v;
    float* q = d ? p1 : p0;
    if (q) q[off] = accumulate ? q[off] + v : v;
  }
}
__global__ void permute_bias_kernel(const float* __restrict__ bi0, const float* __restrict__ bh0,
                                    const float* __restrict__ bi1, const float* __restrict__ bh1, int H, int ngate,
                                    int gru, float* __restrict__ out) {
  const int idx = blockIdx.x * 256 + threadIdx.x;
  const int d = blockIdx.y;
  if (idx >= 4 * H) return;
  const int g = idx & 3, src = g * H + (idx >> 2);
  float v = 0.f;
  if (g < ngate) {
    const float bi = d ? bi1[src] : bi0[src], bh = d ? bh1[src] : bh0[src];
    v = (gru && g == 2) ? bi : bi + bh;
  }
  out[d * 4 * H + idx] = v;
}

inline bool use_hp(int T, int B, int I, int H, int D) {
  if (getenv("RNNT_GEMM_NO_HP")) return false;
  const long M = (long)T * B, N4 = (long)D * 4 * H;
  const long Iw = I > D * H ? I : (long)D * H;
  const size_t lim = (size_t)1 << 32;
  if (hp_plane_bytes(M, Iw) >= lim || hp_plane_bytes(Iw, M) >= lim || hp_plane_bytes(M, N4) >= lim || hp_plane_bytes(N4, M) >= lim ||
      hp_plane_bytes(H, M) >= lim)
    return false;
  return M >= 1024 && N4 >= 512 && H >= 128 && (getenv("RNNT_GEMM_FORCE_HP") || (M * N4 >= (1l << 22)));
}

enum class Form { NONE, V1, V2, V34, V5 };

struct LayerPlan {
  bool accepted;
  Form form;
  Plan v1;
  Plan2 p2;
  bool hp;
  bool takes_row_idx;
  bool takes_f16;
  int recurrence_xcds;
  int cus;
  size_t nflags, hx_bytes;
};

inline int cus_or_mi355x() {
  const int cus = device_cus();
  return cus > 0 ? cus : 256;
}

LayerPlan resolve_plan(int T, int B, int I, int H, int D, int cell, int cus) {
  LayerPlan lp = {};
  lp.form = Form::NONE;
  lp.recurrence_xcds = 8;
  lp.cus = cus;
  if (T < 1 || B < 1 || I < 1 || H < 4 || D < 1 || D > 2) return lp;
  lp.accepted = make_plan(B, H, D, cus, &lp.v1);
  Plan2 v2, v34;
  const bool has2 = make_plan2(B, H, D, cus, &v2), has34 = make_plan3(B, H, D, cus, &v34);
  if (has34) {
    lp.p2 = v34;
    lp.form = lstm5_supported(T, B, H, D, cell) ? Form::V5 : Form::V34;
  } else if (has2) {
    lp.p2 = v2;
    lp.form = Form::V2;
  } else if (lp.accepted && cell == RNNT_CELL_LSTM) {
    lp.form = Form::V1;
  }
  lp.hp = use_hp(T, B, I, H, D);
  lp.takes_f16 = lp.hp && lp.form == Form::V5;
  lp.takes_row_idx = lp.takes_f16 && I >= 32 && T > 1;
  if (lp.form == Form::V5) {
    const int NG = D * lp.p2.G;
    lp.recurrence_xcds = (NG <= 4 && lp.p2.NC <= 32 && !getenv("RNNT_LSTM_NO_XCD_STRIDE")) ? NG : 8;
  }
  auto widen = [&](size_t nflags, size_t hx_bytes) {
    if (nflags > lp.nflags) lp.nflags = nflags;
    if (hx_bytes > lp.hx_bytes) lp.hx_bytes = hx_bytes;
  };
  if (lp.accepted) widen((size_t)D * lp.v1.NC, (size_t)2 * D * H * lp.v1.Bp * 4 * 4);
  if (has2) widen((size_t)D * v2.G * v2.NC, (size_t)2 * D * v2.G * 4 * v2.BQ * 4 * v2.Kp * 4);
  if (has34) {
    widen((size_t)D * v34.G * v34.NC, (size_t)2 * D * v34.G * 4 * v34.BQ * v34.Kp * 6);
    widen((size_t)D * v34.G * v34.NC, (size_t)2 * D * v34.G * v34.NC * 4 * v34.BQ * v34.Kp * 4);
  }
  return lp;
}

struct LstmWs {
  unsigned* flags;
  size_t sync_bytes, nflags;
  float* hx;
  size_t hx_bytes;
  float* wp;
  float* bp;
  float* dwhh;
  unsigned long long* dbg;
  float* dbp;
  size_t dbp_half;
  void* scratch;
  size_t scratch_bytes;
  bool hp;
  char* hp_x;
  char* hp_w;
  char* hp_dg;
  char* hp_dgt;
  char* hp_yt;
  uint32_t* amax_x;
  uint32_t* amax_w;
  uint32_t* amax_dg_rows;
  uint32_t* amax_dg_cols;
  uint32_t* amax_wt;
  uint32_t* amax_xt;
  uint32_t* amax_yt;
  uint32_t* amax_dgh_cols;
  size_t total;
};

LstmWs carve_lstm(void* ws, int T, int B, int I, int H, int D, const LayerPlan& lp) {
  LstmWs w;
  char* p = reinterpret_cast<char*>(ws);
  size_t off = 0;
  auto take = [&](size_t bytes) { char* q = p ? p + off : nullptr; off += align_up(bytes, 256); return q; };
  w.nflags = lp.nflags;
  w.sync_bytes = align_up((2 * w.nflags + 16) * 4, 16);
  w.flags = reinterpret_cast<unsigned*>(take(w.sync_bytes));
  w.hx_bytes = lp.hx_bytes;
  w.hx = reinterpret_cast<float*>(take(w.hx_bytes));
  w.wp = reinterpret_cast<float*>(take((size_t)D * 4 * H * I * 4));
  w.bp = reinterpret_cast<float*>(take((size_t)D * 4 * H * 4));
  w.dwhh = reinterpret_cast<float*>(take((size_t)D * 4 * H * H * 4));
  w.dbg = reinterpret_cast<unsigned long long*>(take(512 * 8 * 8));
  w.dbp_half = (size_t)D * (B + 64) * 4 * H;
  w.dbp = reinterpret_cast<float*>(take(2 * w.dbp_half * 4));
  const int64_t M = (int64_t)T * B, N4 = (int64_t)D * 4 * H;
  size_t sc = rnnt_hip_gemm_workspace_bytes(N4, I, M);
  const size_t s2 = rnnt_hip_gemm_workspace_bytes(4 * H, H, M > B ? M - B : 1);
  const size_t s3 = rnnt_hip_colsum_workspace_bytes(M, N4);
  if (s2 > sc) sc = s2;
  if (s3 > sc) sc = s3;
  w.hp = lp.hp;
  if (w.hp) {
    const size_t h1 = hp_gemm_workspace_bytes(N4, I, M), h2 = hp_gemm_workspace_bytes(4 * H, H, M);
    if (h1 > sc) sc = h1;
    if (h2 > sc) sc = h2;
    const int64_t mn[3] = {N4 * I, (int64_t)4 * H * H, (int64_t)4 * H * H};
    const size_t h3 = HPQ_HEADER_BYTES + hp_gemm_grouped_workspace_bytes(mn, 1 + D);
    if (h3 > sc) sc = h3;
  }
  w.scratch_bytes = sc;
  w.scratch = take(sc);
  w.hp_x = w.hp_w = w.hp_dg = w.hp_dgt = w.hp_yt = nullptr;
  w.amax_x = w.amax_w = w.amax_dg_rows = w.amax_dg_cols = w.amax_wt = w.amax_xt = w.amax_yt = w.amax_dgh_cols = nullptr;
  if (w.hp) {
    uint32_t* hp_amax = reinterpret_cast<uint32_t*>(take((size_t)(2 * M + 3 * N4 + 2 * I + (int64_t)D * H) * 4));
    if (hp_amax) {
      w.amax_x = hp_amax;
      w.amax_w = hp_amax + M;
      w.amax_dg_rows = hp_amax + M + N4;
      w.amax_dg_cols = hp_amax + 2 * M + N4;
      w.amax_wt = hp_amax + 2 * M + 2 * N4;
      w.amax_xt = hp_amax + 2 * M + 2 * N4 + I;
      w.amax_yt = hp_amax + 2 * M + 2 * N4 + 2 * I;
      w.amax_dgh_cols = hp_amax + 2 * M + 2 * N4 + 2 * I + (int64_t)D * H;
    }
    w.hp_x = take(hp_plane_bytes(M, I) > hp_plane_bytes(I, M) ? hp_plane_bytes(M, I) : hp_plane_bytes(I, M));
    w.hp_w = take(hp_plane_bytes(N4, I) > hp_plane_bytes(I, N4) ? hp_plane_bytes(N4, I) : hp_plane_bytes(I, N4));
    w.hp_dg = take(hp_plane_bytes(M, N4));
    w.hp_dgt = take(hp_plane_bytes(N4, M));
    w.hp_yt = take((size_t)D * hp_plane_bytes(H, M));
  }
  w.total = off;
  return w;
}

int check_desc(const rnnt_lstm_desc* d, LayerPlan* lp, LstmWs* w) {
  RNNT_CHECK_ARG(d != nullptr, "lstm: null descriptor");
  RNNT_CHECK_ARG(d->T >= 1 && d->I >= 1, "lstm: T and I must be positive (T=%d I=%d)", d->T, d->I);
  const int cus = device_cus();
  RNNT_CHECK_ARG(cus > 0, "lstm: no HIP device");
  *lp = resolve_plan(d->T, d->B, d->I, d->H, d->D, d->cell, cus);
  if (!lp->accepted) {
    set_error("lstm: unsupported configuration B=%d H=%d D=%d (need H%%4==0, 1<=B<=64, D in {1,2}, slice must fit %d CUs)",
              d->B, d->H, d->D, cus);
    return RNNT_ERR_UNSUPPORTED;
  }
  RNNT_CHECK_ARG(d->cell >= RNNT_CELL_LSTM && d->cell <= RNNT_CELL_RNN_RELU, "lstm: unknown cell type %d", d->cell);
  RNNT_CHECK_ARG(d->lens && d->x && d->y && d->gates && (d->cst || d->cell != RNNT_CELL_LSTM), "lstm: null tensor");
  for (int k = 0; k < d->D; ++k)
    RNNT_CHECK_ARG(d->w_ih[k] && d->w_hh[k] && d->b_ih[k] && d->b_hh[k], "lstm: null weight (direction %d)", k);
  RNNT_CHECK_ARG(d->dropout_p >= 0.f && d->dropout_p < 1.f, "lstm: dropout_p must be in [0,1)");
  RNNT_CHECK_ARG(d->dropout_p == 0.f || d->y_drop, "lstm: dropout_p > 0 needs y_drop");
  RNNT_CHECK_ARG(d->x_abs_bound >= 0.f && d->x_abs_bound < 1e30f, "lstm: x_abs_bound must be 0 (measure) or a finite positive bound");
  RNNT_CHECK_ARG(!d->row_idx || (d->n_rows >= 1 && d->n_rows <= (int64_t)d->T * d->B), "lstm: row_idx needs 1 <= n_rows <= T*B (got %d)", d->n_rows);
  *w = carve_lstm(d->workspace, d->T, d->B, d->I, d->H, d->D, *lp);
  RNNT_CHECK_ARG(d->workspace && d->workspace_bytes >= w->total, "lstm: workspace too small (%zu < %zu)",
                 d->workspace_bytes, w->total);
  RNNT_CHECK_ARG((reinterpret_cast<uintptr_t>(d->gates) & 15) == 0 && (reinterpret_cast<uintptr_t>(d->y) & 15) == 0 &&
                     (reinterpret_cast<uintptr_t>(d->cst) & 15) == 0 && (reinterpret_cast<uintptr_t>(d->aux) & 15) == 0 &&
                     (reinterpret_cast<uintptr_t>(d->workspace) & 255) == 0,
                 "lstm: gates/y/cst must be 16-byte aligned, workspace 256-byte aligned");
  return RNNT_OK;
}

template <class P>
P second(P const (&x)[2], int D) { return D > 1 ? x[1] : x[0]; }

inline int gate_count(int cell) { return cell == RNNT_CELL_LSTM ? 4 : (cell == RNNT_CELL_GRU ? 3 : 1); }

inline bool x_is_plain(const rnnt_lstm_desc* d) { return d->x_sb == d->I && d->x_st == (int64_t)d->B * d->I; }

inline bool ragged_call(const rnnt_lstm_desc* d, const LayerPlan& lp) {
  return d->row_idx && d->n_rows > 0 && d->n_rows < (int64_t)d->T * d->B && x_is_plain(d) && lp.takes_row_idx;
}

void fill_kernel_args(const rnnt_lstm_desc* d, const LayerPlan& lp, const LstmWs& w, LstmK* k) {
  k->T = d->T; k->B = d->B; k->H = d->H; k->D = d->D;
  k->Bp = lp.v1.Bp; k->LDW = lp.v1.LDW;
  if (lp.form == Form::V2 || lp.form == Form::V34 || lp.form == Form::V5) {
    k->NC = lp.p2.NC; k->Hs = lp.p2.HS; k->G = lp.p2.G; k->Bg = lp.p2.Bg; k->Kp = lp.p2.Kp;
  } else {
    k->NC = lp.v1.NC; k->Hs = lp.v1.Hs; k->G = 1; k->Bg = d->B; k->Kp = d->H;
  }
  k->lens = d->lens; k->gates = d->gates; k->cst = d->cst; k->y = d->y;
  k->ydrop = d->dropout_p > 0.f ? d->y_drop : nullptr;
  k->keep_scale = d->dropout_p > 0.f ? 1.f / (1.f - d->dropout_p) : 1.f;
  k->drop_thresh = (unsigned)((double)d->dropout_p * 4294967296.0);
  k->seed = d->dropout_seed;
  k->w_hh[0] = d->w_hh[0]; k->w_hh[1] = second(d->w_hh, d->D);
  k->hx = w.hx; k->status = d->status ? d->status : w.flags; k->flags = w.flags + 16;
  k->dy = nullptr;
  k->cell = d->cell;
  k->b_hh[0] = d->b_hh[0]; k->b_hh[1] = second(d->b_hh, d->D);
  k->aux = d->aux;
  k->NGL = d->D;
  k->dbp = w.dbp; k->dbhp = w.dbp + w.dbp_half;
  k->dbg = getenv("RNNT_LSTM_DBG") ? w.dbg : nullptr;
  k->xcc = w.flags + 16 + w.nflags;
  k->allow_local = getenv("RNNT_LSTM_NO_XCD_LOCAL") ? 0 : 1;
  k->hw_math = getenv("RNNT_LSTM_EXACT_MATH") ? 0 : 1;
  k->pause = 0;
  k->gbound = 0;
  k->colmax = k->colmax_h = nullptr;
  k->rowmax = nullptr;
}

int launch_recurrence(const LayerPlan& lp, const LstmK& k, bool backward, bool f16, hipStream_t s) {
  switch (lp.form) {
    case Form::V5:
      return backward ? lstm5_bwd_launch(k, lp.p2, k.cell, s, f16) : lstm5_fwd_launch(k, lp.p2, k.cell, s, f16);
    case Form::V34:
      return backward ? lstm4_bwd_launch(k, lp.p2, k.cell, s) : lstm3_fwd_launch(k, lp.p2, k.cell, s);
    case Form::V2:
      return backward ? lstm2_bwd_launch(k, lp.p2, k.cell, s) : lstm2_fwd_launch(k, lp.p2, k.cell, s);
    case Form::V1:
      return backward ? lstm1_bwd_launch(k, lp.v1, s) : lstm1_fwd_launch(k, lp.v1, s);
    case Form::NONE:
      break;
  }
  if (backward) set_error("rnn: GRU / Elman cells need the grouped decomposition; B=%d H=%d does not fit", k.B, k.H);
  else set_error("rnn: GRU / Elman cells need the grouped decomposition (B/G <= 16 rows per group); B=%d H=%d does not fit", k.B, k.H);
  return RNNT_ERR_UNSUPPORTED;
}

int reset_exchange(const LstmWs& w, hipStream_t s) {
  RNNT_CHECK_HIP(hipMemsetAsync(w.flags, 0, (size_t)(reinterpret_cast<char*>(w.hx) - reinterpret_cast<char*>(w.flags)) + w.hx_bytes, s));
  return RNNT_OK;
}

int permute_w_ih(const rnnt_lstm_desc* d, const LstmWs& w, hipStream_t s) {
  const long per = (long)4 * d->H * d->I;
  hipLaunchKernelGGL(permute_w_kernel, dim3((unsigned)ceil_div(per, 256), d->D), dim3(256), 0, s, d->w_ih[0], second(d->w_ih, d->D),
                     d->H, d->I, gate_count(d->cell), w.wp);
  RNNT_CHECK_LAUNCH();
  return RNNT_OK;
}

int unpermute(const float* in, int H, int I, int D, int ngate, float* const (&out)[2], int acc, hipStream_t s, float* twin0 = nullptr,
              float* twin1 = nullptr) {
  const long per = (long)4 * H * I;
  hipLaunchKernelGGL(unpermute_w_kernel, dim3((unsigned)ceil_div(per, 256), D), dim3(256), 0, s, in, H, I, per, ngate, out[0],
                     second(out, D), acc, twin0, twin1);
  RNNT_CHECK_LAUNCH();
  return RNNT_OK;
}

}
}

using namespace rnnt;


extern "C" int32_t rnnt_hip_lstm_max_batch(int32_t H, int32_t D, int32_t cell) {
  const int cus = cus_or_mi355x();
  for (int B = 64; B >= 1; --B)
    if (resolve_plan(1, B, 1, H, D, cell, cus).form != Form::NONE) return B;
  return 0;
}

extern "C" int32_t rnnt_hip_lstm_takes_row_idx(int32_t T, int32_t B, int32_t I, int32_t H, int32_t D, int32_t cell) {
  return resolve_plan(T, B, I, H, D, cell, cus_or_mi355x()).takes_row_idx ? 1 : 0;
}

extern "C" int32_t rnnt_hip_lstm_takes_f16(int32_t T, int32_t B, int32_t I, int32_t H, int32_t D, int32_t cell) {
  return resolve_plan(T, B, I, H, D, cell, cus_or_mi355x()).takes_f16 ? 1 : 0;
}

extern "C" int32_t rnnt_hip_lstm_free_xcds(int32_t T, int32_t B, int32_t H, int32_t D, int32_t cell) {
  return 8 - resolve_plan(T, B, 1, H, D, cell, cus_or_mi355x()).recurrence_xcds;
}

extern "C" size_t rnnt_hip_lstm_workspace_bytes(int32_t T, int32_t B, int32_t I, int32_t H, int32_t D) {
  const LayerPlan lp = resolve_plan(T, B, I, H, D, RNNT_CELL_LSTM, cus_or_mi355x());
  return lp.accepted ? carve_lstm(nullptr, T, B, I, H, D, lp).total : 0;
}

static int lstm_fwd_impl(const rnnt_lstm_desc* d, uint32_t precision, void* stream) {
  LayerPlan lp;
  LstmWs w;
  if (int rc = check_desc(d, &lp, &w)) return rc;
  hipStream_t s = (hipStream_t)stream;
  const int H = d->H, D = d->D, I = d->I;
  const int64_t M = (int64_t)d->T * d->B, N4 = (int64_t)D * 4 * H;
  const bool f16 = precision == RNNT_PRECISION_F16 && lp.takes_f16;
  const unsigned hpf = f16 ? RNNT_GEMM_HP_F16 : 0u;
  const bool ragged = ragged_call(d, lp);
  const bool hp_proj = w.hp && x_is_plain(d) && I >= 32;

  if (int rc = permute_w_ih(d, w, s)) return rc;
  hipLaunchKernelGGL(permute_bias_kernel, dim3((unsigned)ceil_div(4 * H, 256), D), dim3(256), 0, s, d->b_ih[0], d->b_hh[0],
                     second(d->b_ih, D), second(d->b_hh, D), H, gate_count(d->cell), d->cell == RNNT_CELL_GRU ? 1 : 0, w.bp);
  RNNT_CHECK_LAUNCH();
  if (hp_proj) {
    const int64_t Mv = ragged ? d->n_rows : M;
    const int* ridx = ragged ? d->row_idx : nullptr;
    if (int rc = hp_split(d->x, Mv, I, I, w.amax_x, w.hp_x, s, ridx)) return rc;
    if (int rc = hp_split(w.wp, N4, I, I, w.amax_w, w.hp_w, s)) return rc;
    if (int rc = hp_gemm(w.hp_x, w.amax_x, w.hp_w, w.amax_w, Mv, N4, I, d->gates, 1, N4, 0, w.bp, hpf, nullptr, 0, s, ridx, M, ridx)) return rc;
  } else {
    rnnt_gemm_desc g = {};
    g.M = M; g.N = N4; g.K = I;
    g.A = d->x; g.a_div = d->B; g.a_so = d->x_st; g.a_si = d->x_sb; g.a_sk = 1; g.a_mc = 0;
    g.B = w.wp; g.b_sn = I; g.b_sk = 1;
    g.C = d->gates; g.c_div = 1; g.c_so = g.N; g.c_si = 0;
    g.bias = w.bp;
    if (int rc = rnnt_hip_gemm_f32(&g, s)) return rc;
  }
  if (int rc = reset_exchange(w, s)) return rc;
  LstmK k;
  fill_kernel_args(d, lp, w, &k);
  k.gbound = ragged ? 1 : 0;
  return launch_recurrence(lp, k, false, f16, s);
}

extern "C" int rnnt_hip_lstm_fwd(const rnnt_lstm_desc* d, void* stream) { return lstm_fwd_impl(d, RNNT_PRECISION_FP32, stream); }

extern "C" int rnnt_hip_lstm_fwd_ex(const rnnt_lstm_desc* d, uint32_t precision, void* stream) {
  RNNT_CHECK_ARG(precision == RNNT_PRECISION_FP32 || precision == RNNT_PRECISION_F16, "lstm_fwd_ex: precision must be 0 (fp32) or 1 (f16), got %u",
                 precision);
  return lstm_fwd_impl(d, precision, stream);
}

static int lstm_bwd_impl(const rnnt_lstm_bwd_desc* bd, uint32_t precision, void* stream) {
  RNNT_CHECK_ARG(bd != nullptr, "lstm_bwd: null descriptor");
  const rnnt_lstm_desc* d = &bd->f;
  LayerPlan lp;
  LstmWs w;
  if (int rc = check_desc(d, &lp, &w)) return rc;
  RNNT_CHECK_ARG(bd->dy, "lstm_bwd: null dy");
  const int T = d->T, B = d->B, H = d->H, D = d->D, I = d->I;
  const bool gru = d->cell == RNNT_CELL_GRU;
  const int ngate = gate_count(d->cell);
  RNNT_CHECK_ARG(!gru || d->aux, "lstm_bwd: GRU needs the aux buffer (T,B,D*4H)");
  for (int k = 0; k < D; ++k) RNNT_CHECK_ARG(!gru || bd->db_hh[k], "lstm_bwd: GRU needs db_hh");
  const int acc = bd->accumulate ? 1 : 0;
  float* twin0 = gru ? nullptr : bd->db_hh[0];
  float* twin1 = gru ? nullptr : second(bd->db_hh, D);
  if (twin0 == bd->db[0]) twin0 = nullptr;
  if (twin1 == second(bd->db, D)) twin1 = nullptr;
  const float* ghid = gru ? d->aux : d->gates;
  RNNT_CHECK_ARG(x_is_plain(d), "lstm_bwd: x must be time-major contiguous (T,B,I)");
  for (int k = 0; k < D; ++k) RNNT_CHECK_ARG(bd->dw_ih[k] && bd->dw_hh[k] && bd->db[k], "lstm_bwd: null gradient output");
  hipStream_t s = (hipStream_t)stream;
  RNNT_CHECK_ARG(bd->phase >= RNNT_LSTM_BWD_ALL && bd->phase <= RNNT_LSTM_BWD_WEIGHTS, "lstm_bwd: phase must be 0, 1 or 2");
  const bool do_recur = bd->phase != RNNT_LSTM_BWD_WEIGHTS, do_weights = bd->phase != RNNT_LSTM_BWD_RECUR;

  const bool f16 = precision == RNNT_PRECISION_F16 && lp.takes_f16;
  const unsigned hpf = f16 ? RNNT_GEMM_HP_F16 : 0u;
  const bool ragged = ragged_call(d, lp);
  const int* ridx = ragged ? d->row_idx : nullptr;
  const int64_t M = (int64_t)T * B, N4 = (int64_t)D * 4 * H;
  const int64_t Mv = ragged ? d->n_rows : M;
  const bool hp_in = w.hp && I >= 128;
  const bool hp_dwih = hp_in || (w.hp && I >= 32 && !getenv("RNNT_GEMM_HP_NO_NARROW"));
  const bool fused_db = lp.form == Form::V34 || lp.form == Form::V5;
  const int db_rows = lp.p2.G * 4 * lp.p2.BQ;
  const bool v5_maxima = lp.form == Form::V5 && w.hp;
  const bool both = v5_maxima && !gru && hp_in && bd->dx && !getenv("RNNT_GEMM_HP_NO_FUSED_SPLIT");
  const unsigned xcd_skip =
      (lp.form == Form::V5 && bd->beside_recurrence && lp.recurrence_xcds <= 4 && lp.cus == 256) ? (1u << lp.recurrence_xcds) - 1u : 0u;
  const bool grouped = hp_in && T > 1 && !gru && (xcd_skip != 0u || getenv("RNNT_GEMM_HP_GROUP")) && !getenv("RNNT_GEMM_HP_NO_GROUP");
  int rc = RNNT_OK;

  if (do_recur)
    if ((rc = reset_exchange(w, s))) return rc;
  LstmK k;
  fill_kernel_args(d, lp, w, &k);
  k.dy = bd->dy;
  k.gbound = ragged ? 1 : 0;
  if (v5_maxima) {
    k.colmax = w.amax_dg_cols;
    k.colmax_h = w.amax_dgh_cols;
    if (both) k.rowmax = w.amax_dg_rows;
    unsigned* first = both ? k.rowmax : k.colmax;
    if (do_recur) RNNT_CHECK_HIP(hipMemsetAsync(first, 0, (size_t)(w.amax_dgh_cols + N4 - first) * 4, s));
  }
  if (do_recur || lp.form == Form::NONE)
    if ((rc = launch_recurrence(lp, k, true, f16, s))) return rc;

  if (w.hp) {
    if (do_recur && hp_in && bd->dx) {
      if (both) rc = hp_split_both(d->gates, Mv, N4, N4, w.amax_dg_rows, w.amax_dg_cols, w.hp_dg, w.hp_dgt, s, ridx);
      else rc = hp_split(d->gates, Mv, N4, N4, w.amax_dg_rows, w.hp_dg, s, ridx);
      if (rc) return rc;
    }
    if (do_weights && !v5_maxima)
      if ((rc = hp_colmax(d->gates, M, N4, N4, w.amax_dg_cols, s))) return rc;
    if (do_weights && !both)
      if ((rc = hp_split_t(d->gates, N4, Mv, N4, M, 0, w.amax_dg_cols, w.hp_dgt, s, ridx))) return rc;
  }
  if (do_recur && bd->dx) {
    if ((rc = permute_w_ih(d, w, s))) return rc;
    if (hp_in) {
      if ((rc = hp_colmax(w.wp, N4, I, I, w.amax_wt, s))) return rc;
      if ((rc = hp_split_t(w.wp, I, N4, I, N4, 0, w.amax_wt, w.hp_w, s))) return rc;
      if ((rc = hp_gemm(w.hp_dg, w.amax_dg_rows, w.hp_w, w.amax_wt, Mv, I, N4, bd->dx, 1, I, 0, nullptr, hpf, nullptr, 0, s, ridx, M, ridx))) return rc;
    } else {
      rnnt_gemm_desc g = {};
      g.M = M; g.N = I; g.K = N4;
      g.A = d->gates; g.a_div = 1; g.a_so = N4; g.a_si = 0; g.a_sk = 1; g.a_mc = 0;
      g.B = w.wp; g.b_sn = 1; g.b_sk = I;
      g.C = bd->dx; g.c_div = 1; g.c_so = I; g.c_si = 0;
      if ((rc = rnnt_hip_gemm_f32(&g, s))) return rc;
    }
    if (ragged) {
      hipLaunchKernelGGL(zero_padded_rows_kernel, dim3((unsigned)(ceil_div(M, 4) < 2048 ? ceil_div(M, 4) : 2048)), dim3(256), 0, s, bd->dx, d->lens, T, B, I);
      RNNT_CHECK_LAUNCH();
    }
  }
  if (!do_weights) return RNNT_OK;
  if (hp_dwih) {
    if (d->x_abs_bound > 0.f) {
      uint32_t bits;
      memcpy(&bits, &d->x_abs_bound, 4);
      RNNT_CHECK_HIP(hipMemsetD32Async((hipDeviceptr_t)w.amax_xt, (int)bits, (size_t)I, s));
    } else if ((rc = hp_colmax(d->x, M, I, I, w.amax_xt, s))) return rc;
    if ((rc = hp_split_t(d->x, I, Mv, I, M, 0, w.amax_xt, w.hp_x, s, ridx))) return rc;
    if (!grouped)
      if ((rc = hp_gemm(w.hp_dgt, w.amax_dg_cols, w.hp_x, w.amax_xt, N4, I, Mv, w.wp, 1, I, 0, nullptr, hpf, w.scratch, w.scratch_bytes, s))) return rc;
  } else {
    rnnt_gemm_desc g = {};
    g.M = N4; g.N = I; g.K = M;
    g.A = d->gates; g.a_mc = 1; g.a_sk = N4; g.a_div = 1;
    g.B = d->x; g.b_sn = 1; g.b_sk = I;
    g.C = w.wp; g.c_div = 1; g.c_so = I; g.c_si = 0;
    g.workspace = w.scratch; g.workspace_bytes = w.scratch_bytes;
    if ((rc = rnnt_hip_gemm_f32(&g, s))) return rc;
  }
  if (!grouped)
    if ((rc = unpermute(w.wp, H, I, D, ngate, bd->dw_ih, acc, s))) return rc;
  if (w.hp && T > 1) {
    if (d->cell != RNNT_CELL_RNN_RELU) {
      RNNT_CHECK_HIP(hipMemsetD32Async((hipDeviceptr_t)w.amax_yt, 0x3f800000, (size_t)D * H, s));
    } else if ((rc = hp_colmax(d->y, M, (int64_t)D * H, (int64_t)D * H, w.amax_yt, s))) return rc;
    uint32_t* a_dgh = w.amax_dg_cols;
    if (gru) {
      if (v5_maxima) a_dgh = w.amax_dgh_cols;
      else if ((rc = hp_colmax(ghid, M, N4, N4, a_dgh, s))) return rc;
      if ((rc = hp_split_t(ghid, N4, Mv, N4, M, 0, a_dgh, w.hp_dgt, s, ridx))) return rc;
    }
    HpProblem pr[HP_GROUP_MAX];
    int npr = 0;
    if (grouped) pr[npr++] = HpProblem{w.hp_dgt, w.amax_dg_cols, w.hp_x, w.amax_xt, N4, I, Mv, w.wp, I, hpf};
    for (int dir = 0; dir < D; ++dir) {
      char* yt = w.hp_yt + (size_t)dir * hp_plane_bytes(H, M);
      uint32_t* a_y = w.amax_yt + (int64_t)dir * H;
      float* dwhh = w.dwhh + (int64_t)dir * 4 * H * H;
      if ((rc = hp_split_t(d->y + (int64_t)dir * H, H, Mv, (int64_t)D * H, M, dir == 0 ? -B : B, a_y, yt, s, ridx))) return rc;
      const char* ag = w.hp_dgt + (size_t)dir * 4 * H * (size_t)ceil_div(Mv, 32) * 128;
      if (grouped) {
        pr[npr++] = HpProblem{ag, a_dgh + (int64_t)dir * 4 * H, yt, a_y, 4 * H, H, Mv, dwhh, H, hpf};
        continue;
      }
      if ((rc = hp_gemm(ag, a_dgh + (int64_t)dir * 4 * H, yt, a_y, 4 * H, H, Mv, dwhh, 1, H, 0, nullptr, hpf, w.scratch, w.scratch_bytes, s)))
        return rc;
    }
    if (grouped) {
      if ((rc = hp_gemm_grouped(pr, npr, xcd_skip, reinterpret_cast<unsigned*>(w.scratch), (char*)w.scratch + HPQ_HEADER_BYTES,
                                w.scratch_bytes - HPQ_HEADER_BYTES, s, k.status)))
        return rc;
      if ((rc = unpermute(w.wp, H, I, D, ngate, bd->dw_ih, acc, s))) return rc;
    }
  } else
  for (int dir = 0; dir < D; ++dir) {
    rnnt_gemm_desc g = {};
    g.M = 4 * H; g.N = H; g.K = (int64_t)(T - 1) * B;
    const int64_t shift_g = dir == 0 ? (int64_t)B * N4 : 0;
    const int64_t shift_y = dir == 0 ? 0 : (int64_t)B * D * H;
    g.A = ghid + shift_g + (int64_t)dir * 4 * H; g.a_mc = 1; g.a_sk = N4; g.a_div = 1;
    g.B = d->y + shift_y + (int64_t)dir * H; g.b_sn = 1; g.b_sk = (int64_t)D * H;
    g.C = w.dwhh + (int64_t)dir * 4 * H * H; g.c_div = 1; g.c_so = H; g.c_si = 0;
    g.workspace = w.scratch; g.workspace_bytes = w.scratch_bytes;
    if (g.K > 0) {
      if ((rc = rnnt_hip_gemm_f32(&g, s))) return rc;
    } else {
      RNNT_CHECK_HIP(hipMemsetAsync(g.C, 0, (size_t)4 * H * H * 4, s));
    }
  }
  if ((rc = unpermute(w.dwhh, H, H, D, ngate, bd->dw_hh, acc, s))) return rc;
  if (fused_db) {
    hipLaunchKernelGGL(db_reduce_kernel, dim3((unsigned)ceil_div(4 * H, 256), D), dim3(256), 0, s, k.dbp, db_rows, H, ngate, bd->db[0],
                       second(bd->db, D), acc, twin0, twin1);
    RNNT_CHECK_LAUNCH();
    if (gru) {
      hipLaunchKernelGGL(db_reduce_kernel, dim3((unsigned)ceil_div(4 * H, 256), D), dim3(256), 0, s, k.dbhp, db_rows, H, ngate, bd->db_hh[0],
                         second(bd->db_hh, D), acc);
      RNNT_CHECK_LAUNCH();
    }
  } else {
    if ((rc = launch_colsum(d->gates, (long)M, (long)N4, (long)N4, w.bp, w.scratch, w.scratch_bytes, s))) return rc;
    if ((rc = unpermute(w.bp, H, 1, D, ngate, bd->db, acc, s, twin0, twin1))) return rc;
    if (gru) {
      if ((rc = launch_colsum(ghid, (long)M, (long)N4, (long)N4, w.bp, w.scratch, w.scratch_bytes, s))) return rc;
      if ((rc = unpermute(w.bp, H, 1, D, ngate, bd->db_hh, acc, s))) return rc;
    }
  }
  return RNNT_OK;
}

extern "C" int rnnt_hip_lstm_bwd(const rnnt_lstm_bwd_desc* bd, void* stream) { return lstm_bwd_impl(bd, RNNT_PRECISION_FP32, stream); }

extern "C" int rnnt_hip_lstm_bwd_ex(const rnnt_lstm_bwd_desc* bd, uint32_t precision, void* stream) {
  RNNT_CHECK_ARG(precision == RNNT_PRECISION_FP32 || precision == RNNT_PRECISION_F16, "lstm_bwd_ex: precision must be 0 (fp32) or 1 (f16), got %u",
                 precision);
  return lstm_bwd_impl(bd, precision, stream);
}

extern "C" int rnnt_hip_lstm_check(const void* workspace, void* stream) {
  RNNT_CHECK_ARG(workspace != nullptr, "lstm_check: null workspace");
  unsigned st = 0;
  RNNT_CHECK_HIP(hipMemcpyAsync(&st, workspace, sizeof(st), hipMemcpyDeviceToHost, (hipStream_t)stream));
  RNNT_CHECK_HIP(hipStreamSynchronize((hipStream_t)stream));
  if (st != 0) {
    set_error("persistent LSTM kernel abandoned an inter-workgroup wait (status %u)", st);
    return RNNT_ERR_TIMEOUT;
  }
  return RNNT_OK;
}

extern "C" int rnnt_hip_lstm_debug_read(const void* workspace, int32_t T, int32_t B, int32_t I, int32_t H, int32_t D,
                                        uint64_t* out, int32_t nwg, void* stream) {
  RNNT_CHECK_ARG(workspace && out && nwg >= 1 && nwg <= 512, "lstm_debug_read: bad arguments");
  const LayerPlan lp = resolve_plan(T, B, I, H, D, RNNT_CELL_LSTM, device_cus());
  RNNT_CHECK_ARG(lp.accepted, "lstm_debug_read: unsupported shape");
  const LstmWs w = carve_lstm(const_cast<void*>(workspace), T, B, I, H, D, lp);
  RNNT_CHECK_HIP(hipMemcpyAsync(out, w.dbg, (size_t)nwg * 8 * 8, hipMemcpyDeviceToHost, (hipStream_t)stream));
  RNNT_CHECK_HIP(hipStreamSynchronize((hipStream_t)stream));
  return RNNT_OK;
}
```

Before: 1272.

## Fuse weight permute/split prep kernels and fold unpermute into split-K GEMM epilogue

Adds fused kernels that permute and hp-split the input weights directly from the original layout, for both forward and transposed backward use. The backward one also fills the constant amax tables that were previously set with memsets. The split-K reduction epilogue of the hp GEMM can now scatter into gate-unpermuted dW outputs, with accumulate and twin copies, so the separate unpermute pass is skipped. The GRU bias reductions are merged into one launch and the exchange reset absorbs an amax memset. This removes several small launches and intermediate round-trips through memory, at the cost of more complex kernels and less coalesced scattered epilogue writes.

New measurement: 1270. No clear change (-0.1%).

```diff
diff --git a/include/rnnt_hip.h b/include/rnnt_hip.h
--- a/include/rnnt_hip.h
+++ b/include/rnnt_hip.h
@@ -80,6 +80,9 @@
                       void* planes, uint32_t* amax, int32_t amax_given, void* stream);
 int rnnt_hip_hp_split_both(const float* x, int64_t M, int64_t C, int64_t ld, const uint32_t* rowmax, const uint32_t* colmax,
                            void* planes_rm, void* planes_t, void* stream);
+int rnnt_hip_hp_prepare_w(const float* w_ih0, const float* w_ih1, const float* b_ih0, const float* b_hh0, const float* b_ih1,
+                          const float* b_hh1, int32_t H, int32_t I, int32_t D, int32_t cell, int32_t transpose, void* planes,
+                          uint32_t* amax, float* bias, void* stream);
 size_t rnnt_hip_gemm_hp_workspace_bytes(int64_t M, int64_t N, int64_t K);
 int rnnt_hip_gemm_hp(const void* A, const uint32_t* a_amax, const void* B, const uint32_t* b_amax, int64_t M, int64_t N, int64_t K,
                      float* C, int64_t ldc, const float* bias, uint32_t flags, void* workspace, size_t workspace_bytes,
@@ -155,6 +158,9 @@
 
 int rnnt_hip_lstm_bwd(const rnnt_lstm_bwd_desc* d, void* stream);
 int rnnt_hip_lstm_bwd_ex(const rnnt_lstm_bwd_desc* d, uint32_t precision, void* stream);
+int rnnt_hip_lstm_dw_finish(const void* A, const uint32_t* a_amax, const void* B, const uint32_t* b_amax, int64_t M, int64_t N, int64_t K,
+                            int32_t H, int32_t ngate, float* out0, float* out1, float* twin0, float* twin1, int32_t accumulate,
+                            int32_t direct, float* scratch, void* workspace, size_t workspace_bytes, int32_t* mapped, void* stream);
 int rnnt_hip_lstm_check(const void* workspace, void* stream);
 int rnnt_hip_lstm_debug_read(const void* workspace, int32_t T, int32_t B, int32_t I, int32_t H, int32_t D,
                              uint64_t* out, int32_t nwg, void* stream);
diff --git a/rnntransducer_amd/_lib.py b/rnntransducer_amd/_lib.py
--- a/rnntransducer_amd/_lib.py
+++ b/rnntransducer_amd/_lib.py
@@ -145,6 +145,7 @@
     "rnnt_hip_gemm_plan": (C.c_int, [C.POINTER(GemmDesc), C.POINTER(GemmPlan)]),
     "rnnt_hip_hp_bytes": (C.c_size_t, [c_i64, c_i64]),
     "rnnt_hip_hp_split": (C.c_int, [C.c_void_p, c_i64, c_i64, c_i64, c_i32, c_i64, c_i64, C.c_void_p, C.c_void_p, c_i32, C.c_void_p]),
+    "rnnt_hip_hp_prepare_w": (C.c_int, [C.c_void_p] * 6 + [c_i32] * 5 + [C.c_void_p] * 4),
     "rnnt_hip_gemm_hp_workspace_bytes": (C.c_size_t, [c_i64, c_i64, c_i64]),
     "rnnt_hip_gemm_hp": (C.c_int, [C.c_void_p, C.c_void_p, C.c_void_p, C.c_void_p, c_i64, c_i64, c_i64, C.c_void_p, c_i64, C.c_void_p,
                                   C.c_uint32, C.c_void_p, C.c_size_t, C.c_void_p]),
@@ -160,6 +161,8 @@
     "rnnt_hip_lstm_takes_f16": (c_i32, [c_i32] * 6),
     "rnnt_hip_lstm_bwd": (C.c_int, [C.POINTER(LstmBwdDesc), C.c_void_p]),
     "rnnt_hip_lstm_bwd_ex": (C.c_int, [C.POINTER(LstmBwdDesc), C.c_uint32, C.c_void_p]),
+    "rnnt_hip_lstm_dw_finish": (C.c_int, [C.c_void_p] * 4 + [c_i64] * 3 + [c_i32] * 2 + [C.c_void_p] * 4 + [c_i32] * 2 +
+                                [C.c_void_p, C.c_void_p, C.c_size_t, C.c_void_p, C.c_void_p]),
     "rnnt_hip_lstm_check": (C.c_int, [C.c_void_p, C.c_void_p]),
     "rnnt_hip_lstm_debug_read": (C.c_int, [C.c_void_p, c_i32, c_i32, c_i32, c_i32, c_i32, C.c_void_p, c_i32, C.c_void_p]),
     "rnnt_hip_joint_loss_workspace_bytes": (C.c_size_t, [c_i32] * 4),
diff --git a/rnntransducer_amd/csrc/common.hpp b/rnntransducer_amd/csrc/common.hpp
--- a/rnntransducer_amd/csrc/common.hpp
+++ b/rnntransducer_amd/csrc/common.hpp
@@ -54,10 +54,20 @@
                hipStream_t s, const int* kidx = nullptr);
 int hp_split_both(const float* x, int64_t M, int64_t C, int64_t ld, const uint32_t* rowmax, const uint32_t* colmax, void* planes_rm,
                   void* planes_t, hipStream_t s, const int* rowidx = nullptr);
+int hp_prepare_w_fwd(const float* const (&w_ih)[2], const float* const (&b_ih)[2], const float* const (&b_hh)[2], int H, int I, int D, int ngate,
+                     int gru, uint32_t* amax, void* planes, float* bias, hipStream_t s);
+int hp_prepare_w_bwd(const float* const (&w_ih)[2], int H, int I, int D, int ngate, uint32_t* amax_wt, void* planes, uint32_t* fill_a,
+                     uint32_t a_bits, int64_t a_n, uint32_t* fill_b, uint32_t b_bits, int64_t b_n, hipStream_t s);
+struct HpRowMap {
+  int H, ngate, accumulate;
+  float* out[2];
+  float* twin[2];
+};
 size_t hp_gemm_workspace_bytes(int64_t M, int64_t N, int64_t K);
 int hp_gemm(const void* A, const uint32_t* a_amax, const void* B, const uint32_t* b_amax, int64_t M, int64_t N, int64_t K, float* C,
             int64_t c_div, int64_t c_so, int64_t c_si, const float* bias, unsigned flags, void* workspace, size_t workspace_bytes,
-            hipStream_t s, const int* a_rowidx = nullptr, int64_t a_plane_rows = 0, const int* c_rowidx = nullptr);
+            hipStream_t s, const int* a_rowidx = nullptr, int64_t a_plane_rows = 0, const int* c_rowidx = nullptr,
+            const HpRowMap* map = nullptr, bool* mapped = nullptr);
 struct HpProblem {
   const void* A; const uint32_t* a_amax; const void* B; const uint32_t* b_amax;
   int64_t M, N, K;
diff --git a/rnntransducer_amd/csrc/gemm_hp.hip b/rnntransducer_amd/csrc/gemm_hp.hip
--- a/rnntransducer_amd/csrc/gemm_hp.hip
+++ b/rnntransducer_amd/csrc/gemm_hp.hip
@@ -48,47 +48,147 @@
   lo = __builtin_bit_cast(u32x4, l);
 }
 
+__device__ __forceinline__ void hp_split_row(const float* __restrict__ row, int K, bool vec, int lane, unsigned* __restrict__ amax_r,
+                                             char* __restrict__ out_row) {
+  const int Kp = (K + 31) & ~31, cpr = Kp >> 3;
+  unsigned m = 0;
+  if (row)
+    for (int c = lane; c < cpr; c += 64) {
+      const int k = 8 * c;
+      if (vec && k + 7 < K) {
+        const u32x4 a = *reinterpret_cast<const u32x4*>(row + k), b = *reinterpret_cast<const u32x4*>(row + k + 4);
+#pragma unroll
+        for (int e = 0; e < 4; ++e) m = max(m, max(a[e] & 0x7fffffffu, b[e] & 0x7fffffffu));
+      } else {
+#pragma unroll
+        for (int e = 0; e < 8; ++e)
+          if (k + e < K) m = max(m, __float_as_uint(row[k + e]) & 0x7fffffffu);
+      }
+    }
+#pragma unroll
+  for (int o = 32; o > 0; o >>= 1) m = max(m, (unsigned)__shfl_xor((int)m, o));
+  if (lane == 0) *amax_r = m;
+  const float scale = hp_scale_from_amax(m);
+  for (int c = lane; c < cpr; c += 64) {
+    const int k = 8 * c;
+    float v[8];
+    if (!row) {
+#pragma unroll
+      for (int e = 0; e < 8; ++e) v[e] = 0.f;
+    } else if (vec && k + 7 < K) {
+      const f32x4 a = *reinterpret_cast<const f32x4*>(row + k), b = *reinterpret_cast<const f32x4*>(row + k + 4);
+      v[0] = a[0]; v[1] = a[1]; v[2] = a[2]; v[3] = a[3]; v[4] = b[0]; v[5] = b[1]; v[6] = b[2]; v[7] = b[3];
+    } else {
+#pragma unroll
+      for (int e = 0; e < 8; ++e) v[e] = (k + e < K) ? row[k + e] : 0.f;
+    }
+    u32x4 hi, lo;
+    hp_split8(v, scale, hi, lo);
+    char* dst = out_row + (long)(c >> 2) * 128 + 16 * (c & 3);
+    *reinterpret_cast<u32x4*>(dst) = hi;
+    *reinterpret_cast<u32x4*>(dst + 64) = lo;
+  }
+}
+
 __global__ void __launch_bounds__(256) hp_split_kernel(const float* __restrict__ x, long rows, int K, long ld, unsigned* __restrict__ amax,
                                                        char* __restrict__ out, const int* __restrict__ rowidx) {
-  const int Kp = (K + 31) & ~31, cpr = Kp >> 3;
+  const long pitch = (long)((K + 31) >> 5) * 128;
   const int lane = threadIdx.x & 63;
   const bool vec = (ld & 3) == 0 && (reinterpret_cast<uintptr_t>(x) & 15) == 0;
   for (long ri = (long)blockIdx.x * 4 + (threadIdx.x >> 6); ri < rows; ri += (long)gridDim.x * 4) {
     const long r = rowidx ? (long)rowidx[ri] : ri;
-    const float* row = x + r * ld;
-    unsigned m = 0;
-    for (int c = lane; c < cpr; c += 64) {
-      const int k = 8 * c;
-      if (vec && k + 7 < K) {
-        const u32x4 a = *reinterpret_cast<const u32x4*>(row + k), b = *reinterpret_cast<const u32x4*>(row + k + 4);
-#pragma unroll
-        for (int e = 0; e < 4; ++e) m = max(m, max(a[e] & 0x7fffffffu, b[e] & 0x7fffffffu));
-      } else {
-#pragma unroll
-        for (int e = 0; e < 8; ++e)
-          if (k + e < K) m = max(m, __float_as_uint(row[k + e]) & 0x7fffffffu);
-      }
-    }
-#pragma unroll
-    for (int o = 32; o > 0; o >>= 1) m = max(m, (unsigned)__shfl_xor((int)m, o));
-    if (lane == 0) amax[r] = m;
-    const float scale = hp_scale_from_amax(m);
-    for (int c = lane; c < cpr; c += 64) {
-      const int k = 8 * c;
-      float v[8];
-      if (vec && k + 7 < K) {
-        const f32x4 a = *reinterpret_cast<const f32x4*>(row + k), b = *reinterpret_cast<const f32x4*>(row + k + 4);
-        v[0] = a[0]; v[1] = a[1]; v[2] = a[2]; v[3] = a[3]; v[4] = b[0]; v[5] = b[1]; v[6] = b[2]; v[7] = b[3];
-      } else {
-#pragma unroll
-        for (int e = 0; e < 8; ++e) v[e] = (k + e < K) ? row[k + e] : 0.f;
-      }
-      u32x4 hi, lo;
-      hp_split8(v, scale, hi, lo);
-      char* dst = out + (r * (Kp >> 5) + (c >> 2)) * 128 + 16 * (c & 3);
-      *reinterpret_cast<u32x4*>(dst) = hi;
-      *reinterpret_cast<u32x4*>(dst + 64) = lo;
-    }
+    hp_split_row(x + r * ld, K, vec, lane, amax + r, out + r * pitch);
+  }
+}
+
+__global__ void __launch_bounds__(256) hp_prepare_w_fwd_kernel(const float* __restrict__ w0, const float* __restrict__ w1,
+                                                               const float* __restrict__ bi0, const float* __restrict__ bh0,
+                                                               const float* __restrict__ bi1, const float* __restrict__ bh1, int H, int I,
+                                                               int ngate, int gru, unsigned* __restrict__ amax, char* __restrict__ out,
+                                                               float* __restrict__ bp) {
+  const int lane = threadIdx.x & 63, d = blockIdx.y;
+  const int r = blockIdx.x * 4 + (threadIdx.x >> 6);
+  if (r >= 4 * H) return;
+  const int g = r & 3, src = g * H + (r >> 2);
+  const float* w = d ? w1 : w0;
+  const bool vec = (I & 3) == 0 && (reinterpret_cast<uintptr_t>(w) & 15) == 0;
+  const long ro = (long)d * 4 * H + r;
+  hp_split_row(g < ngate ? w + (long)src * I : nullptr, I, vec, lane, amax + ro, out + ro * ((long)((I + 31) >> 5) * 128));
+  if (lane == 0) {
+    float v = 0.f;
+    if (g < ngate) {
+      const float bi = d ? bi1[src] : bi0[src], bh = d ? bh1[src] : bh0[src];
+      v = (gru && g == 2) ? bi : bi + bh;
+    }
+    bp[ro] = v;
+  }
+}
+
+constexpr int HP_PW_COLS = 32, HP_PW_K = 128;
+__global__ void __launch_bounds__(1024) hp_prepare_w_bwd_kernel(const float* __restrict__ w0, const float* __restrict__ w1, int H, int I, int D,
+                                                                int ngate, unsigned* __restrict__ amax_wt, char* __restrict__ out,
+                                                                unsigned* __restrict__ fill_a, unsigned a_bits, int a_n,
+                                                                unsigned* __restrict__ fill_b, unsigned b_bits, int b_n) {
+  __shared__ float tile[HP_PW_K][HP_PW_COLS + 1];
+  __shared__ unsigned smax[HP_PW_COLS];
+  const int tid = threadIdx.x;
+  for (int i = blockIdx.x * 1024 + tid; i < a_n; i += gridDim.x * 1024) fill_a[i] = a_bits;
+  for (int i = blockIdx.x * 1024 + tid; i < b_n; i += gridDim.x * 1024) fill_b[i] = b_bits;
+  if (tid < HP_PW_COLS) smax[tid] = 0u;
+  __syncthreads();
+  const int i0 = blockIdx.x * HP_PW_COLS, N4 = D * 4 * H;
+  const int kr = tid >> 3, cl = 4 * (tid & 7), c = i0 + cl;
+  const bool vec = (I & 3) == 0 && ((reinterpret_cast<uintptr_t>(w0) | reinterpret_cast<uintptr_t>(w1)) & 15) == 0;
+  auto load = [&](int k) {
+    f32x4 v = {0.f, 0.f, 0.f, 0.f};
+    if (k < N4 && c < I) {
+      const int d = k / (4 * H), r = k - d * 4 * H;
+      if ((r & 3) < ngate) {
+        const float* src = (d ? w1 : w0) + (long)((r & 3) * H + (r >> 2)) * I + c;
+        if (vec && c + 3 < I) {
+          v = *reinterpret_cast<const f32x4*>(src);
+        } else {
+#pragma unroll
+          for (int e = 0; e < 4; ++e)
+            if (c + e < I) v[e] = src[e];
+        }
+      }
+    }
+    return v;
+  };
+  unsigned m[4] = {0u, 0u, 0u, 0u};
+#pragma unroll 4
+  for (int k = kr; k < N4; k += HP_PW_K) {
+    const f32x4 v = load(k);
+#pragma unroll
+    for (int e = 0; e < 4; ++e) m[e] = max(m[e], __float_as_uint(v[e]) & 0x7fffffffu);
+  }
+#pragma unroll
+  for (int e = 0; e < 4; ++e)
+    if (m[e] != 0u) atomicMax(&smax[cl + e], m[e]);
+  __syncthreads();
+  if (tid < HP_PW_COLS && i0 + tid < I) amax_wt[i0 + tid] = smax[tid];
+  const int Kp32 = (N4 + 31) >> 5;
+  for (int k0 = 0; k0 < Kp32 * 32; k0 += HP_PW_K) {
+    const f32x4 v = load(k0 + kr);
+#pragma unroll
+    for (int e = 0; e < 4; ++e) tile[kr][cl + e] = v[e];
+    __syncthreads();
+    if (tid < 512) {
+      const int kbl = tid >> 7, rl = (tid >> 2) & 31, ch = tid & 3;
+      const int kb = (k0 >> 5) + kbl;
+      if (kb < Kp32 && i0 + rl < I) {
+        float x[8];
+#pragma unroll
+        for (int e = 0; e < 8; ++e) x[e] = tile[32 * kbl + 8 * ch + e][rl];
+        u32x4 hi, lo;
+        hp_split8(x, hp_scale_from_amax(smax[rl]), hi, lo);
+        char* dst = out + ((long)(i0 + rl) * Kp32 + kb) * 128 + 16 * ch;
+        *reinterpret_cast<u32x4*>(dst) = hi;
+        *reinterpret_cast<u32x4*>(dst + 64) = lo;
+      }
+    }
+    __syncthreads();
   }
 }
 
@@ -204,6 +304,7 @@
   int group_m;
   const int* a_rowidx;
   const int* c_rowidx;
+  HpRowMap map;
 };
 
 __device__ __forceinline__ int hp_xcd_remap(int bid, int n) {
@@ -427,6 +528,16 @@
     const int m = (int)(i / p.N), n = (int)(i % p.N);
     float s = 0.f;
     for (int z = 0; z < p.splits; ++z) s += p.slab[(long)z * total + i];
+    if (p.map.H > 0) {
+      const int d = m / (4 * p.map.H), r = m - d * 4 * p.map.H;
+      if ((r & 3) >= p.map.ngate) continue;
+      const long off = (long)((r & 3) * p.map.H + (r >> 2)) * p.N + n;
+      float* o = p.map.out[d];
+      o[off] = p.map.accumulate ? o[off] + s : s;
+      float* q = p.map.twin[d];
+      if (q) q[off] = p.map.accumulate ? q[off] + s : s;
+      continue;
+    }
     if (p.bias) s += p.bias[n];
     const int mo = p.c_rowidx ? p.c_rowidx[m] : m;
     const long off = (long)(mo / p.c_div) * p.c_so + (long)(mo % p.c_div) * p.c_si + n;
@@ -483,6 +594,24 @@
   return RNNT_OK;
 }
 
+int hp_prepare_w_fwd(const float* const (&w_ih)[2], const float* const (&b_ih)[2], const float* const (&b_hh)[2], int H, int I, int D, int ngate,
+                     int gru, uint32_t* amax, void* planes, float* bias, hipStream_t s) {
+  ProfScope prof(RNNT_K_HP_SPLIT, 8.0 * (double)D * 4 * H * (double)I, s);
+  hipLaunchKernelGGL(hp_prepare_w_fwd_kernel, dim3((unsigned)H, (unsigned)D), dim3(256), 0, s, w_ih[0], w_ih[D - 1], b_ih[0], b_hh[0], b_ih[D - 1],
+                     b_hh[D - 1], H, I, ngate, gru, amax, (char*)planes, bias);
+  RNNT_CHECK_LAUNCH();
+  return RNNT_OK;
+}
+
+int hp_prepare_w_bwd(const float* const (&w_ih)[2], int H, int I, int D, int ngate, uint32_t* amax_wt, void* planes, uint32_t* fill_a,
+                     uint32_t a_bits, int64_t a_n, uint32_t* fill_b, uint32_t b_bits, int64_t b_n, hipStream_t s) {
+  ProfScope prof(RNNT_K_HP_SPLIT, 12.0 * (double)D * 4 * H * (double)I, s);
+  hipLaunchKernelGGL(hp_prepare_w_bwd_kernel, dim3((unsigned)ceil_div(I, HP_PW_COLS)), dim3(1024), 0, s, w_ih[0], w_ih[D - 1], H, I, D, ngate,
+                     amax_wt, (char*)planes, fill_a, a_bits, (int)(fill_a ? a_n : 0), fill_b, b_bits, (int)(fill_b ? b_n : 0));
+  RNNT_CHECK_LAUNCH();
+  return RNNT_OK;
+}
+
 size_t hp_gemm_workspace_bytes(int64_t M, int64_t N, int64_t K) {
   const long tiles = ceil_div(M, HP_BM) * ceil_div(N, HP_BN);
   const long nkt = ceil_div(K, HP_BK);
@@ -495,8 +624,11 @@
 
 int hp_gemm(const void* A, const uint32_t* a_amax, const void* B, const uint32_t* b_amax, int64_t M, int64_t N, int64_t K, float* C,
             int64_t c_div, int64_t c_so, int64_t c_si, const float* bias, unsigned flags, void* workspace, size_t workspace_bytes,
-            hipStream_t s, const int* a_rowidx, int64_t a_plane_rows, const int* c_rowidx) {
+            hipStream_t s, const int* a_rowidx, int64_t a_plane_rows, const int* c_rowidx, const HpRowMap* map, bool* mapped) {
   RNNT_CHECK_ARG(A && B && C && a_amax && b_amax, "gemm_hp: null operand");
+  RNNT_CHECK_ARG(!map || (mapped && map->H >= 1 && M % (4 * map->H) == 0 && M / (4 * map->H) <= 2 && !bias && !c_rowidx),
+                 "gemm_hp: a row map takes M = D*4H rows (D <= 2), no bias, no output scatter");
+  if (mapped) *mapped = false;
   RNNT_CHECK_ARG(!a_rowidx || a_plane_rows >= M, "gemm_hp: a gathered A operand needs the row count of its planes");
   RNNT_CHECK_ARG(M >= 1 && N >= 1 && K >= 1 && M < (1ll << 31) && N < (1ll << 31) && K < (1ll << 31), "gemm_hp: bad dims");
   RNNT_CHECK_ARG(c_div >= 1, "gemm_hp: c_div must be >= 1");
@@ -511,6 +643,7 @@
   k.C = C; k.c_div = (int)(c_div > 0x7fffffff ? 0x7fffffff : c_div); k.c_so = c_so; k.c_si = c_si;
   k.bias = bias; k.flags = flags;
   k.a_rowidx = a_rowidx; k.c_rowidx = c_rowidx;
+  k.map = HpRowMap{};
   const bool f16 = (flags & RNNT_GEMM_HP_F16) != 0u;
   k.tiles_m = (int)ceil_div(M, HP_BM); k.tiles_n = (int)ceil_div(N, HP_BN);
   const int tiles = k.tiles_m * k.tiles_n;
@@ -531,6 +664,10 @@
   splits = (int)ceil_div(k.nkt, k.kt_per_split);
   k.splits = splits;
   k.slab = (float*)workspace;
+  if (map && splits > 1) {
+    k.map = *map;
+    *mapped = true;
+  }
   if (f16) RNNT_CHECK_HIP(hipFuncSetAttribute((const void*)gemm_hp_kernel<true>, hipFuncAttributeMaxDynamicSharedMemorySize, 2 * HP_STAGE));
   else RNNT_CHECK_HIP(hipFuncSetAttribute((const void*)gemm_hp_kernel<false>, hipFuncAttributeMaxDynamicSharedMemorySize, 2 * HP_STAGE));
   {
@@ -654,6 +791,21 @@
   return hp_split_t(x, rows, K, ld, src_rows, shift, amax, planes, s);
 }
 
+extern "C" int rnnt_hip_hp_prepare_w(const float* w_ih0, const float* w_ih1, const float* b_ih0, const float* b_hh0, const float* b_ih1,
+                                     const float* b_hh1, int32_t H, int32_t I, int32_t D, int32_t cell, int32_t transpose, void* planes,
+                                     uint32_t* amax, float* bias, void* stream) {
+  RNNT_CHECK_ARG(H >= 1 && I >= 1 && (D == 1 || D == 2) && cell >= RNNT_CELL_LSTM && cell <= RNNT_CELL_RNN_RELU, "hp_prepare_w: bad shape");
+  RNNT_CHECK_ARG(w_ih0 && (D == 1 || w_ih1) && planes && amax, "hp_prepare_w: null tensor");
+  RNNT_CHECK_ARG((reinterpret_cast<uintptr_t>(planes) & 127) == 0, "hp_prepare_w: planes must be 128-byte aligned");
+  const int ngate = cell == RNNT_CELL_LSTM ? 4 : (cell == RNNT_CELL_GRU ? 3 : 1);
+  const float* const w[2] = {w_ih0, D > 1 ? w_ih1 : w_ih0};
+  if (transpose) return hp_prepare_w_bwd(w, H, I, D, ngate, amax, planes, nullptr, 0u, 0, nullptr, 0u, 0, (hipStream_t)stream);
+  RNNT_CHECK_ARG(bias && b_ih0 && b_hh0 && (D == 1 || (b_ih1 && b_hh1)), "hp_prepare_w: null bias");
+  const float* const bi[2] = {b_ih0, D > 1 ? b_ih1 : b_ih0};
+  const float* const bh[2] = {b_hh0, D > 1 ? b_hh1 : b_hh0};
+  return hp_prepare_w_fwd(w, bi, bh, H, I, D, ngate, cell == RNNT_CELL_GRU ? 1 : 0, amax, planes, bias, (hipStream_t)stream);
+}
+
 extern "C" size_t rnnt_hip_gemm_hp_workspace_bytes(int64_t M, int64_t N, int64_t K) {
   if (M < 1 || N < 1 || K < 1) return 0;
   return hp_gemm_workspace_bytes(M, N, K);
diff --git a/rnntransducer_amd/csrc/lstm_layer.hip b/rnntransducer_amd/csrc/lstm_layer.hip
--- a/rnntransducer_amd/csrc/lstm_layer.hip
+++ b/rnntransducer_amd/csrc/lstm_layer.hip
@@ -6,10 +6,13 @@
 namespace {
 
 __global__ void db_reduce_kernel(const float* __restrict__ part, int rows_per_dir, int H, int ngate, float* __restrict__ o0,
-                                 float* __restrict__ o1, int accumulate, float* __restrict__ p0 = nullptr,
-                                 float* __restrict__ p1 = nullptr) {
+                                 float* __restrict__ o1, int accumulate, float* __restrict__ p0, float* __restrict__ p1,
+                                 const float* __restrict__ part_h, float* __restrict__ h0, float* __restrict__ h1) {
   const int c = blockIdx.x * 256 + threadIdx.x, d = blockIdx.y;
   if (c >= 4 * H || (c & 3) >= ngate) return;
+  if (blockIdx.z) {
+    part = part_h; o0 = h0; o1 = h1; p0 = p1 = nullptr;
+  }
   const float* src = part + (long)d * rows_per_dir * 4 * H + c;
   float s = 0.f;
   for (int r = 0; r < rows_per_dir; ++r) s += src[(long)r * 4 * H];
@@ -161,14 +164,14 @@
   char* hp_dg;
   char* hp_dgt;
   char* hp_yt;
-  uint32_t* amax_x;
-  uint32_t* amax_w;
   uint32_t* amax_dg_rows;
   uint32_t* amax_dg_cols;
   uint32_t* amax_wt;
   uint32_t* amax_xt;
   uint32_t* amax_yt;
   uint32_t* amax_dgh_cols;
+  uint32_t* amax_x;
+  uint32_t* amax_w;
   size_t total;
 };
 
@@ -182,19 +185,33 @@
   w.flags = reinterpret_cast<unsigned*>(take(w.sync_bytes));
   w.hx_bytes = lp.hx_bytes;
   w.hx = reinterpret_cast<float*>(take(w.hx_bytes));
+  const int64_t M = (int64_t)T * B, N4 = (int64_t)D * 4 * H;
+  w.hp = lp.hp;
+  w.amax_x = w.amax_w = w.amax_dg_rows = w.amax_dg_cols = w.amax_wt = w.amax_xt = w.amax_yt = w.amax_dgh_cols = nullptr;
+  if (w.hp) {
+    uint32_t* hp_amax = reinterpret_cast<uint32_t*>(take((size_t)(2 * M + 3 * N4 + 2 * I + (int64_t)D * H) * 4));
+    if (hp_amax) {
+      w.amax_dg_rows = hp_amax;
+      w.amax_dg_cols = w.amax_dg_rows + M;
+      w.amax_wt = w.amax_dg_cols + N4;
+      w.amax_xt = w.amax_wt + I;
+      w.amax_yt = w.amax_xt + I;
+      w.amax_dgh_cols = w.amax_yt + (int64_t)D * H;
+      w.amax_x = w.amax_dgh_cols + N4;
+      w.amax_w = w.amax_x + M;
+    }
+  }
   w.wp = reinterpret_cast<float*>(take((size_t)D * 4 * H * I * 4));
   w.bp = reinterpret_cast<float*>(take((size_t)D * 4 * H * 4));
   w.dwhh = reinterpret_cast<float*>(take((size_t)D * 4 * H * H * 4));
   w.dbg = reinterpret_cast<unsigned long long*>(take(512 * 8 * 8));
   w.dbp_half = (size_t)D * (B + 64) * 4 * H;
   w.dbp = reinterpret_cast<float*>(take(2 * w.dbp_half * 4));
-  const int64_t M = (int64_t)T * B, N4 = (int64_t)D * 4 * H;
   size_t sc = rnnt_hip_gemm_workspace_bytes(N4, I, M);
   const size_t s2 = rnnt_hip_gemm_workspace_bytes(4 * H, H, M > B ? M - B : 1);
   const size_t s3 = rnnt_hip_colsum_workspace_bytes(M, N4);
   if (s2 > sc) sc = s2;
   if (s3 > sc) sc = s3;
-  w.hp = lp.hp;
   if (w.hp) {
     const size_t h1 = hp_gemm_workspace_bytes(N4, I, M), h2 = hp_gemm_workspace_bytes(4 * H, H, M);
     if (h1 > sc) sc = h1;
@@ -206,19 +223,7 @@
   w.scratch_bytes = sc;
   w.scratch = take(sc);
   w.hp_x = w.hp_w = w.hp_dg = w.hp_dgt = w.hp_yt = nullptr;
-  w.amax_x = w.amax_w = w.amax_dg_rows = w.amax_dg_cols = w.amax_wt = w.amax_xt = w.amax_yt = w.amax_dgh_cols = nullptr;
   if (w.hp) {
-    uint32_t* hp_amax = reinterpret_cast<uint32_t*>(take((size_t)(2 * M + 3 * N4 + 2 * I + (int64_t)D * H) * 4));
-    if (hp_amax) {
-      w.amax_x = hp_amax;
-      w.amax_w = hp_amax + M;
-      w.amax_dg_rows = hp_amax + M + N4;
-      w.amax_dg_cols = hp_amax + 2 * M + N4;
-      w.amax_wt = hp_amax + 2 * M + 2 * N4;
-      w.amax_xt = hp_amax + 2 * M + 2 * N4 + I;
-      w.amax_yt = hp_amax + 2 * M + 2 * N4 + 2 * I;
-      w.amax_dgh_cols = hp_amax + 2 * M + 2 * N4 + 2 * I + (int64_t)D * H;
-    }
     w.hp_x = take(hp_plane_bytes(M, I) > hp_plane_bytes(I, M) ? hp_plane_bytes(M, I) : hp_plane_bytes(I, M));
     w.hp_w = take(hp_plane_bytes(N4, I) > hp_plane_bytes(I, N4) ? hp_plane_bytes(N4, I) : hp_plane_bytes(I, N4));
     w.hp_dg = take(hp_plane_bytes(M, N4));
@@ -318,8 +323,9 @@
   return RNNT_ERR_UNSUPPORTED;
 }
 
-int reset_exchange(const LstmWs& w, hipStream_t s) {
-  RNNT_CHECK_HIP(hipMemsetAsync(w.flags, 0, (size_t)(reinterpret_cast<char*>(w.hx) - reinterpret_cast<char*>(w.flags)) + w.hx_bytes, s));
+int reset_exchange(const LstmWs& w, hipStream_t s, bool with_maxima = false, int64_t N4 = 0) {
+  const char* end = with_maxima ? reinterpret_cast<const char*>(w.amax_dgh_cols + N4) : reinterpret_cast<const char*>(w.hx) + w.hx_bytes;
+  RNNT_CHECK_HIP(hipMemsetAsync(w.flags, 0, (size_t)(end - reinterpret_cast<const char*>(w.flags)), s));
   return RNNT_OK;
 }
 
@@ -382,17 +388,18 @@
   const bool ragged = ragged_call(d, lp);
   const bool hp_proj = w.hp && x_is_plain(d) && I >= 32;
 
-  if (int rc = permute_w_ih(d, w, s)) return rc;
-  hipLaunchKernelGGL(permute_bias_kernel, dim3((unsigned)ceil_div(4 * H, 256), D), dim3(256), 0, s, d->b_ih[0], d->b_hh[0],
-                     second(d->b_ih, D), second(d->b_hh, D), H, gate_count(d->cell), d->cell == RNNT_CELL_GRU ? 1 : 0, w.bp);
-  RNNT_CHECK_LAUNCH();
   if (hp_proj) {
     const int64_t Mv = ragged ? d->n_rows : M;
     const int* ridx = ragged ? d->row_idx : nullptr;
+    if (int rc = hp_prepare_w_fwd(d->w_ih, d->b_ih, d->b_hh, H, I, D, gate_count(d->cell), d->cell == RNNT_CELL_GRU ? 1 : 0, w.amax_w, w.hp_w, w.bp, s))
+      return rc;
     if (int rc = hp_split(d->x, Mv, I, I, w.amax_x, w.hp_x, s, ridx)) return rc;
-    if (int rc = hp_split(w.wp, N4, I, I, w.amax_w, w.hp_w, s)) return rc;
     if (int rc = hp_gemm(w.hp_x, w.amax_x, w.hp_w, w.amax_w, Mv, N4, I, d->gates, 1, N4, 0, w.bp, hpf, nullptr, 0, s, ridx, M, ridx)) return rc;
   } else {
+    if (int rc = permute_w_ih(d, w, s)) return rc;
+    hipLaunchKernelGGL(permute_bias_kernel, dim3((unsigned)ceil_div(4 * H, 256), D), dim3(256), 0, s, d->b_ih[0], d->b_hh[0],
+                       second(d->b_ih, D), second(d->b_hh, D), H, gate_count(d->cell), d->cell == RNNT_CELL_GRU ? 1 : 0, w.bp);
+    RNNT_CHECK_LAUNCH();
     rnnt_gemm_desc g = {};
     g.M = M; g.N = N4; g.K = I;
     g.A = d->x; g.a_div = d->B; g.a_so = d->x_st; g.a_si = d->x_sb; g.a_sk = 1; g.a_mc = 0;
@@ -458,7 +465,7 @@
   int rc = RNNT_OK;
 
   if (do_recur)
-    if ((rc = reset_exchange(w, s))) return rc;
+    if ((rc = reset_exchange(w, s, v5_maxima, N4))) return rc;
   LstmK k;
   fill_kernel_args(d, lp, w, &k);
   k.dy = bd->dy;
@@ -467,8 +474,6 @@
     k.colmax = w.amax_dg_cols;
     k.colmax_h = w.amax_dgh_cols;
     if (both) k.rowmax = w.amax_dg_rows;
-    unsigned* first = both ? k.rowmax : k.colmax;
-    if (do_recur) RNNT_CHECK_HIP(hipMemsetAsync(first, 0, (size_t)(w.amax_dgh_cols + N4 - first) * 4, s));
   }
   if (do_recur || lp.form == Form::NONE)
     if ((rc = launch_recurrence(lp, k, true, f16, s))) return rc;
@@ -484,13 +489,18 @@
     if (do_weights && !both)
       if ((rc = hp_split_t(d->gates, N4, Mv, N4, M, 0, w.amax_dg_cols, w.hp_dgt, s, ridx))) return rc;
   }
+  const bool xt_const = hp_dwih && d->x_abs_bound > 0.f, yt_const = w.hp && T > 1 && d->cell != RNNT_CELL_RNN_RELU;
+  const bool tables_by_prepare = bd->dx && hp_in;
+  uint32_t xt_bits;
+  memcpy(&xt_bits, &d->x_abs_bound, 4);
   if (do_recur && bd->dx) {
-    if ((rc = permute_w_ih(d, w, s))) return rc;
     if (hp_in) {
-      if ((rc = hp_colmax(w.wp, N4, I, I, w.amax_wt, s))) return rc;
-      if ((rc = hp_split_t(w.wp, I, N4, I, N4, 0, w.amax_wt, w.hp_w, s))) return rc;
+      if ((rc = hp_prepare_w_bwd(d->w_ih, H, I, D, ngate, w.amax_wt, w.hp_w, xt_const ? w.amax_xt : nullptr, xt_bits, I,
+                                 yt_const ? w.amax_yt : nullptr, 0x3f800000u, (int64_t)D * H, s)))
+        return rc;
       if ((rc = hp_gemm(w.hp_dg, w.amax_dg_rows, w.hp_w, w.amax_wt, Mv, I, N4, bd->dx, 1, I, 0, nullptr, hpf, nullptr, 0, s, ridx, M, ridx))) return rc;
     } else {
+      if ((rc = permute_w_ih(d, w, s))) return rc;
       rnnt_gemm_desc g = {};
       g.M = M; g.N = I; g.K = N4;
       g.A = d->gates; g.a_div = 1; g.a_so = N4; g.a_si = 0; g.a_sk = 1; g.a_mc = 0;
@@ -504,15 +514,18 @@
     }
   }
   if (!do_weights) return RNNT_OK;
+  bool dwih_mapped = false;
   if (hp_dwih) {
-    if (d->x_abs_bound > 0.f) {
-      uint32_t bits;
-      memcpy(&bits, &d->x_abs_bound, 4);
-      RNNT_CHECK_HIP(hipMemsetD32Async((hipDeviceptr_t)w.amax_xt, (int)bits, (size_t)I, s));
+    if (xt_const) {
+      if (!tables_by_prepare) RNNT_CHECK_HIP(hipMemsetD32Async((hipDeviceptr_t)w.amax_xt, (int)xt_bits, (size_t)I, s));
     } else if ((rc = hp_colmax(d->x, M, I, I, w.amax_xt, s))) return rc;
     if ((rc = hp_split_t(d->x, I, Mv, I, M, 0, w.amax_xt, w.hp_x, s, ridx))) return rc;
-    if (!grouped)
-      if ((rc = hp_gemm(w.hp_dgt, w.amax_dg_cols, w.hp_x, w.amax_xt, N4, I, Mv, w.wp, 1, I, 0, nullptr, hpf, w.scratch, w.scratch_bytes, s))) return rc;
+    if (!grouped) {
+      const HpRowMap map = {H, ngate, acc, {bd->dw_ih[0], second(bd->dw_ih, D)}, {nullptr, nullptr}};
+      if ((rc = hp_gemm(w.hp_dgt, w.amax_dg_cols, w.hp_x, w.amax_xt, N4, I, Mv, w.wp, 1, I, 0, nullptr, hpf, w.scratch, w.scratch_bytes, s, nullptr, 0,
+                        nullptr, &map, &dwih_mapped)))
+        return rc;
+    }
   } else {
     rnnt_gemm_desc g = {};
     g.M = N4; g.N = I; g.K = M;
@@ -522,11 +535,12 @@
     g.workspace = w.scratch; g.workspace_bytes = w.scratch_bytes;
     if ((rc = rnnt_hip_gemm_f32(&g, s))) return rc;
   }
-  if (!grouped)
+  if (!grouped && !dwih_mapped)
     if ((rc = unpermute(w.wp, H, I, D, ngate, bd->dw_ih, acc, s))) return rc;
+  bool dwhh_mapped[2] = {false, false};
   if (w.hp && T > 1) {
-    if (d->cell != RNNT_CELL_RNN_RELU) {
-      RNNT_CHECK_HIP(hipMemsetD32Async((hipDeviceptr_t)w.amax_yt, 0x3f800000, (size_t)D * H, s));
+    if (yt_const) {
+      if (!tables_by_prepare) RNNT_CHECK_HIP(hipMemsetD32Async((hipDeviceptr_t)w.amax_yt, 0x3f800000, (size_t)D * H, s));
     } else if ((rc = hp_colmax(d->y, M, (int64_t)D * H, (int64_t)D * H, w.amax_yt, s))) return rc;
     uint32_t* a_dgh = w.amax_dg_cols;
     if (gru) {
@@ -547,7 +561,9 @@
         pr[npr++] = HpProblem{ag, a_dgh + (int64_t)dir * 4 * H, yt, a_y, 4 * H, H, Mv, dwhh, H, hpf};
         continue;
       }
-      if ((rc = hp_gemm(ag, a_dgh + (int64_t)dir * 4 * H, yt, a_y, 4 * H, H, Mv, dwhh, 1, H, 0, nullptr, hpf, w.scratch, w.scratch_bytes, s)))
+      const HpRowMap map = {H, ngate, acc, {bd->dw_hh[dir], nullptr}, {nullptr, nullptr}};
+      if ((rc = hp_gemm(ag, a_dgh + (int64_t)dir * 4 * H, yt, a_y, 4 * H, H, Mv, dwhh, 1, H, 0, nullptr, hpf, w.scratch, w.scratch_bytes, s, nullptr, 0,
+                        nullptr, &map, &dwhh_mapped[dir])))
         return rc;
     }
     if (grouped) {
@@ -572,16 +588,19 @@
       RNNT_CHECK_HIP(hipMemsetAsync(g.C, 0, (size_t)4 * H * H * 4, s));
     }
   }
-  if ((rc = unpermute(w.dwhh, H, H, D, ngate, bd->dw_hh, acc, s))) return rc;
+  if (!dwhh_mapped[0] && !dwhh_mapped[D - 1]) {
+    if ((rc = unpermute(w.dwhh, H, H, D, ngate, bd->dw_hh, acc, s))) return rc;
+  } else {
+    for (int dir = 0; dir < D; ++dir)
+      if (!dwhh_mapped[dir]) {
+        float* const one[2] = {bd->dw_hh[dir], nullptr};
+        if ((rc = unpermute(w.dwhh + (int64_t)dir * 4 * H * H, H, H, 1, ngate, one, acc, s))) return rc;
+      }
+  }
   if (fused_db) {
-    hipLaunchKernelGGL(db_reduce_kernel, dim3((unsigned)ceil_div(4 * H, 256), D), dim3(256), 0, s, k.dbp, db_rows, H, ngate, bd->db[0],
-                       second(bd->db, D), acc, twin0, twin1);
+    hipLaunchKernelGGL(db_reduce_kernel, dim3((unsigned)ceil_div(4 * H, 256), D, gru ? 2 : 1), dim3(256), 0, s, k.dbp, db_rows, H, ngate,
+                       bd->db[0], second(bd->db, D), acc, twin0, twin1, k.dbhp, bd->db_hh[0], second(bd->db_hh, D));
     RNNT_CHECK_LAUNCH();
-    if (gru) {
-      hipLaunchKernelGGL(db_reduce_kernel, dim3((unsigned)ceil_div(4 * H, 256), D), dim3(256), 0, s, k.dbhp, db_rows, H, ngate, bd->db_hh[0],
-                         second(bd->db_hh, D), acc);
-      RNNT_CHECK_LAUNCH();
-    }
   } else {
     if ((rc = launch_colsum(d->gates, (long)M, (long)N4, (long)N4, w.bp, w.scratch, w.scratch_bytes, s))) return rc;
     if ((rc = unpermute(w.bp, H, 1, D, ngate, bd->db, acc, s, twin0, twin1))) return rc;
@@ -599,6 +618,27 @@
   RNNT_CHECK_ARG(precision == RNNT_PRECISION_FP32 || precision == RNNT_PRECISION_F16, "lstm_bwd_ex: precision must be 0 (fp32) or 1 (f16), got %u",
                  precision);
   return lstm_bwd_impl(bd, precision, stream);
+}
+
+extern "C" int rnnt_hip_lstm_dw_finish(const void* A, const uint32_t* a_amax, const void* B, const uint32_t* b_amax, int64_t M, int64_t N, int64_t K,
+                                       int32_t H, int32_t ngate, float* out0, float* out1, float* twin0, float* twin1, int32_t accumulate,
+                                       int32_t direct, float* scratch, void* workspace, size_t workspace_bytes, int32_t* mapped,
+                                       void* stream) {
+  RNNT_CHECK_ARG(H >= 1 && ngate >= 1 && ngate <= 4 && M >= 1 && N >= 1 && M < (1ll << 31) && N < (1ll << 31) && M % (4 * H) == 0 && M / (4 * H) <= 2,
+                 "lstm_dw_finish: M must be D*4H rows, D in {1,2}");
+  const int D = (int)(M / (4 * H));
+  RNNT_CHECK_ARG(out0 && (D == 1 || out1) && scratch && mapped, "lstm_dw_finish: null tensor");
+  hipStream_t s = (hipStream_t)stream;
+  const int acc = accumulate ? 1 : 0;
+  const HpRowMap map = {H, ngate, acc, {out0, out1}, {twin0, twin1}};
+  bool m = false;
+  if (int rc = hp_gemm(A, a_amax, B, b_amax, M, N, K, scratch, 1, N, 0, nullptr, 0u, workspace, workspace_bytes, s, nullptr, 0, nullptr,
+                       direct ? &map : nullptr, direct ? &m : nullptr))
+    return rc;
+  *mapped = m ? 1 : 0;
+  if (m) return RNNT_OK;
+  float* const out[2] = {out0, out1};
+  return unpermute(scratch, H, (int)N, D, ngate, out, acc, s, twin0, twin1);
 }
 
 extern "C" int rnnt_hip_lstm_check(const void* workspace, void* stream) {
```
